# EdwardjkFeng/gradslam

Hardware: AMD Instinct MI355X
Metric: RGB-D frames/sec (640x480, 10 ICP iters) (higher is better)
Workload: dtype f32; 1 GPU; c2: ICP odometry localisation step, 640x480 TUM-shape synthetic RGB-D, batch 1 per GPU, dsratio 4 (~19k x ~19k points), 10 LM iterations, map 288269 points; parallelism=one sequence per GPU, final RCCL all_gather of poses, timing=one timed region of 1356 steps

## Files before the change

gradslam_amd/csrc/gs_drivers.hpp:

```cpp
#pragma once

#include "gs_common.hpp"
#include "gs_project.hpp"

namespace gs {

int vertex_normal_maps_cam(const float *depth, const float *intrinsics, const float *poses, int B, int H, int W, float *vertex,
                           float *normal, float *gvertex, float *gnormal, float *cam_out, hipStream_t st);
int vertex_normal_maps_fusion(const float *depth, const float *intrinsics, const float *poses, int B, int H, int W, float *gvertex,
                              float *gnormal, float *alpha, float sigma, float eps, unsigned long long *pix_key, unsigned int *pix_n,
                              int32_t *zero, int n_zero, hipStream_t st);

constexpr int kBucketPixMax = 24 * 1024;
size_t project_target1_ws_bytes(int H, int W, int ds, int Nmax);
int project_target1(const float *points, const int32_t *counts, int Nmax, const float *poses, const float *intrinsics, int H, int W, int ds,
                    const float *map_normals, int cap, int64_t *rows, int32_t *nrows, float *tgt, float *tnrm, int32_t *nt,
                    float *scan_points, int32_t *scan_orig, int32_t *pix_start, int32_t *tgt_index, int32_t *tgt_pix, void *ws,
                    size_t ws_bytes, hipStream_t st, const DsJob *frame);
int project_front1(const float *depth, const float *points, const int32_t *counts, int Nmax, const float *poses, const float *intrinsics,
                   int H, int W, int ds, const float *map_normals, int cap, float *vertex, float *normal, float *gvertex, float *gnormal,
                   float *cam_out, int32_t *row_pix, float *tgt, float *tnrm, int32_t *nt, int32_t *tgt_index, float *scan_points,
                   int32_t *scan_orig, int32_t *pix_start, const DsJob &frame, void *ws, size_t ws_bytes, hipStream_t st);

size_t fusion_corr_state_bytes(int B, int H, int W, int Nmax);
void fusion_corr_init_ptrs(void *state, int B, int H, int W, int Nmax, unsigned long long **pix_key, unsigned int **pix_n);
int fusion_correspond(void *state, const float *map_points, const float *map_normals, const float *map_ccounts, const int32_t *counts,
                      int B, int Nmax, const float *poses, const float *intrinsics, int H, int W, const float *gvertex,
                      const float *gnormal, float dist_th, float dot_th, int32_t *ctr, hipStream_t st);
int fusion_merge_corr(void *state, const int32_t *ctr, const float *gvertex, const float *gnormal, const float *rgb, const float *alpha,
                      int B, int H, int W, int Nmax, const int32_t *counts, float *points, float *normals, float *colors, float *ccounts,
                      hipStream_t st);
int fusion_append_corr(void *state, int B, int H, int W, int Nmax, int b, const float *depth, const float *const *h_src,
                       const int *h_row_floats, float *const *h_dst, const int32_t *d_count, int cap, int *d_total, void *cws,
                       hipStream_t st);
int fusion_finish(void *state, int B, int H, int W, int Nmax, int32_t *ctr, int32_t *counts, const int *totals, int cap, int32_t *appended,
                  int32_t *stats, hipStream_t st);
size_t append_scratch_bytes(int64_t HW);
size_t fusion_tape_bytes(int B, int H, int W);
int fusion_tape_record(const void *state, void *tape, int B, int H, int W, int Nmax, const int32_t *counts, const float *points,
                       const float *normals, const float *colors, const float *ccounts, hipStream_t st);
int fusion_tape_appended(void *tape, int B, int H, int W, const int32_t *appended, hipStream_t st);
int fusion_update_reverse(const void *tape, int B, int H, int W, int Nmax, const float *depth, const float *gvertex, const float *gnormal,
                          const float *rgb, const float *alpha, float *points, float *normals, float *colors, float *ccounts,
                          int32_t *counts, float *Gp, float *Gn, float *Gc, float *Gcc, float *g_gvertex, float *g_gnormal, float *g_rgb,
                          float *g_alpha, void *cws, hipStream_t st);
int append_valid_pixels(int n_arrays, const float *depth_b, int64_t HW, const float *const *h_src, const int *h_row_floats,
                        float *const *h_dst, int32_t *d_count, int cap, int32_t *d_appended, int32_t *d_overflow, void *cws,
                        hipStream_t st);

}
```

gradslam_amd/csrc/gs_icp_loop.hpp:

```cpp
#pragma once

#include "gs_icp_step.hpp"
#include "gs_project.hpp"

namespace gs {

struct LoopConst {
    const float *user_src, *tgt, *nrm, *boxes, *sboxes;
    const int32_t *d_ns, *d_nt;
    float *trace, *out_T;
    gs_icp_hints hints;
    GradParams gp;
    float thresh;
    int ns, nt;
    int cert_off;
    int tile_points;
    int grid_variant;
    CamK cam;
    int cam_ok;
    int32_t *cells;
    int cells_stride;
};

__device__ __forceinline__ f3 cam_point(const CamK &k, const f3 p) {
// ... 465 lines not shown
        unsigned long long scan_diag = 0;
#endif
        {
            float bd = INFINITY;
            int bi = 0x7fffffff;
            const int2 w0 = sh.wrow[0][lane], w1 = sh.wrow[1][lane], w2 = sh.wrow[2][lane];
            static_assert(WROWS == 3, "the flattened scan names its three rows");
            const int total = w0.y + w1.y + w2.y;
            auto element = [&](const int p) { return lanewin::element(p, w0.y, w1.y, w0.x, w1.x, w2.x); };
            auto take = [&](const float4 q) {
                const float d = dist2(s, q.x, q.y, q.z);
                const int jj = __float_as_int(q.w);
                const bool better = (d < bd) | ((d == bd) & (jj < bi));
                bd = better ? d : bd;
                bi = better ? jj : bi;
            };
#ifdef GS_DIAG_STAMPS
            unsigned int n_iter = 0;
#endif
            const float4 *pool = reinterpret_cast<const float4 *>(sh.u.stage);
            if (!__any((w0.x | w1.x | w2.x) < 0)) {
                for (int p = wave; p < total; p += 2 * NW) {
                    const int ea = element(p), eb = element(min(p + NW, total - 1));
                    const float4 qa = pool[ea], qb = pool[eb];
                    take(qa);
                    take(qb);
#ifdef GS_DIAG_STAMPS
                    ++n_iter;
#endif
                }
            } else {
                for (int p = wave; p < total; p += NW) {
                    const int e = element(p);
                    float4 q;
                    if (e >= 0) {
                        q = pool[e];
                    } else {
                        const int slot = LaneWin::mem_slot(e);
                        const f3 g3 = ld3(C->hints.scan_points, slot);
                        q = make_float4(g3.x, g3.y, g3.z, __int_as_float(C->hints.scan_orig[slot]));
                    }
                    take(q);
#ifdef GS_DIAG_STAMPS
                    ++n_iter;
#endif
                }
            }
            if (ok && bd < INFINITY) atomicMin(&sh.key[lane], pack_key(bd, bi));
#ifdef GS_DIAG_STAMPS
            scan_diag = ((unsigned long long)n_iter << 8) | ((unsigned long long)(unsigned)wave_max_i(total) << 32);
#endif
        }
        __syncthreads();
        GS_STAMP(1);
        float bd;
        int bi;
        key_unpack(sh.key[lane], bd, bi);
        const float bound2 = (ok && C->cam_ok) ? cam_bound2(sh.cam, s, sh.centre[lane], rel >> 3) : 0.0f;
        const bool proven = !C->cert_off & ((rel & 4) != 0) & (bd * 1.0001f < bound2);
        need = ok & !proven;
        unsigned long long need_mask = __ballot(need);
#ifdef GS_DIAG_STAMPS
        GS_COUNT(12, (unsigned long long)__popcll(need_mask) | scan_diag);
#endif
        if constexpr (NW == 8) {
            if (__popcll(need_mask) > 6 && C->cam_ok && !C->cert_off) {
                need = knn_second_window<NW>(sh, s, need, bd, nt, C->hints.pix_start, C->hints.scan_points, C->hints.scan_orig, win2_word);
                need_mask = __ballot(need);
            }
        }
        bool tile_search = __popcll(need_mask) > 6;
        if (!tile_search && need_mask) {
            tile_search = !knn_point_search<NW>(sh, s, need_mask, C->hints.scan_points, C->hints.scan_orig, C->boxes, C->sboxes, nt);
        }
        if (tile_search) {
            tile_box(sh, s, need);
            __syncthreads();
            knn_prune_search<true, NW>(sh, s, ok, need, C->hints.scan_points, C->hints.scan_orig, C->boxes, C->sboxes, nt);
        }
        if constexpr (NW == 8) win2_word |= (unsigned)__popcll(need_mask) | (tile_search ? 0x400u : 0u);
#ifdef GS_DIAG_STAMPS
        if (wave == 0) GS_COUNT(15, (unsigned long long)win2_word);
#endif

        GS_STAMP(2);
        key = ok ? sh.key[lane] : KEY_NONE;
        GS_STAMP(3);
        GS_COUNT(5, ((unsigned long long)__builtin_amdgcn_s_getreg((31 << 11) | 4) << 16) |
                        ((unsigned long long)__builtin_amdgcn_s_getreg((31 << 11) | 20) << 48));
    } else {
        int sj = -1;
        if (!first) {
            sj = -2;
            if (wave == 0) {
                unsigned long long k0 = KEY_NONE;
                if (ok) {
                    const float4 q = *reinterpret_cast<const float4 *>(sh.seed[b_cur == S_in->b_cur ? 0 : 1][lane]);
                    k0 = pack_key(dist2(s, q.x, q.y, q.z), __float_as_int(q.w));
                }
                sh.key[lane] = k0;
            }
        }
        const bool window_seed = first && C->hints.scan_points && C->hints.src_pix && C->hints.pix_start && C->hints.grid_w > 0;
        if (window_seed) sj = -2;
        const float *scan = C->hints.scan_points ? C->hints.scan_points : C->tgt;
        const int32_t *scan_orig = C->hints.scan_points ? C->hints.scan_orig : nullptr;
        if (window_seed) knn_window_seed<NW>(sh, s, ok, i, C->hints, nt);
        key = knn_tile<NW>(sh, s, ok, sj, C->tgt, scan, scan_orig, C->boxes, C->sboxes, nt);
    }
    if (wave == 0) {
        if (ok) best[i] = key;
        if (grid && ok && C->cam_ok) C->cells[par * C->cells_stride + i] = cam_cell(sh.cam, s);
        float acc[NACC];
#pragma unroll
        for (int k = 0; k < NACC; ++k) acc[k] = 0.0f;
        const Row r = make_row_from(s, ok, key, C->tgt, C->nrm, C->thresh);
        if (r.valid) accumulate_row(r, acc);
#pragma unroll
        for (int k = 0; k < NACC; ++k) sh.u.a.rows[k][lane] = acc[k];
    }
    __syncthreads();
    static_assert(NACC * 16 <= NW * 64, "the J epilogue's first stage is one pass");
    if (threadIdx.x < NACC * 16) {
        const int k = threadIdx.x >> 4, p4 = (threadIdx.x & 15) * 4;
        sh.u.a.part[k][threadIdx.x & 15] = ((sh.u.a.rows[k][p4] + sh.u.a.rows[k][p4 + 1]) + sh.u.a.rows[k][p4 + 2]) + sh.u.a.rows[k][p4 + 3];
    }
    __syncthreads();
    if (threadIdx.x < NACC) {
        float v = 0.0f;
#pragma unroll
        for (int q = 0; q < 16; ++q) v += sh.u.a.part[threadIdx.x][q];
        partials[blockIdx.x * NACC + threadIdx.x] = v;
    }
    if constexpr (GRID && NW == 8) {
        if (threadIdx.x == 0 && (win2_word & 0x300u)) window_count(win2_word);
    }
}

__global__ void icp_init_state_k(IcpState *S, const float *__restrict__ init_T , float damp) {
    if (threadIdx.x == 0 && blockIdx.x == 0) {
        for (int i = 0; i < 16; ++i) {
            const float v = init_T ? init_T[i] : ((i % 5 == 0) ? 1.0f : 0.0f);
            S->T[i] = v; S->dT[i] = v;
        }
        for (int i = 0; i < 44; ++i) S->cur[i] = 0.0f;
        S->damp = damp;
        S->p_cur = 1;
        S->b_cur = 1; S->b_first = 0;
        S->it = 0;
    }
}

__global__ __launch_bounds__(SUPER * CHUNK) void icp_prepare_k(IcpState *S, const float *__restrict__ init_T, float damp,
                                                              const float *__restrict__ tgt, const int32_t *__restrict__ d_nt,
                                                              float *__restrict__ boxes, float *__restrict__ sboxes,
                                                              LoopConst lc, LoopConst *__restrict__ lc_out, float *__restrict__ part0,
                                                              float *__restrict__ part1, int rows_written, int rows_read) {
    static_assert(SUPER * CHUNK == 1024, "one block per super-box");
    for (int q = rows_written * NACC + blockIdx.x * blockDim.x + threadIdx.x; q < rows_read * NACC; q += gridDim.x * blockDim.x) {
        part0[q] = 0.0f; part1[q] = 0.0f;
    }
    __shared__ float wb[16][6];
    if (blockIdx.x == 0 && threadIdx.x < sizeof(LoopConst) / 4) {
        int v = reinterpret_cast<const int *>(&lc)[threadIdx.x];
        if (threadIdx.x == offsetof(LoopConst, ns) / 4) v = *lc.d_ns;
        if (threadIdx.x == offsetof(LoopConst, nt) / 4) v = *lc.d_nt;
        if (threadIdx.x == offsetof(LoopConst, tile_points) / 4) {
            atomicAdd(&g_loop_counts[0], 1u);
            if (lc.grid_variant) atomicAdd(&g_loop_counts[1], 1u);
            if (lc.tile_points != 64) atomicAdd(&g_loop_counts[2], 1u);
        }
        reinterpret_cast<int *>(lc_out)[threadIdx.x] = v;
    }
    if (lc.cells) {
        const int n = *lc.d_ns;
        int32_t *pix = lc.cells + 2 * (size_t)lc.cells_stride;
        for (int i = blockIdx.x * blockDim.x + threadIdx.x; i < lc.cells_stride; i += gridDim.x * blockDim.x)
            pix[i] = (i < n && lc.hints.src_pix) ? lc.hints.src_pix[i] : 0;
    }
    if (blockIdx.x == 0) {
        __syncthreads();
        if (threadIdx.x == 0 && lc.hints.cam_pose && lc.hints.cam_K && lc.hints.ds > 0) {
            const float *T = lc.hints.cam_pose, *K = lc.hints.cam_K;
            const Cam c = make_cam(T, K);
            for (int q = 0; q < 9; ++q) lc_out->cam.R[q] = c.R[q];
            for (int q = 0; q < 3; ++q) lc_out->cam.T[q] = c.tinv[q];
            lc_out->cam.fx = K[0]; lc_out->cam.fy = K[5]; lc_out->cam.cx = K[2]; lc_out->cam.cy = K[6];
            lc_out->cam.ds = lc.hints.ds; lc_out->cam.Wd = lc.hints.grid_w; lc_out->cam.Hd = lc.hints.grid_h;
            const bool pinhole = K[1] == 0.0f && K[3] == 0.0f && K[4] == 0.0f && K[7] == 0.0f && K[8] == 0.0f && K[9] == 0.0f &&
                                 K[10] == 1.0f && K[11] == 0.0f && K[0] != 0.0f && K[5] != 0.0f;
            lc_out->cam_ok = pinhole ? 1 : 0;
        }
    }
    if (threadIdx.x == 0 && blockIdx.x == 0) {
        for (int i = 0; i < 16; ++i) {
            const float v = init_T ? init_T[i] : ((i % 5 == 0) ? 1.0f : 0.0f);
            S->T[i] = v; S->dT[i] = v;
        }
        for (int i = 0; i < 44; ++i) S->cur[i] = 0.0f;
        for (int i = 0; i < 6; ++i) S->xi[i] = 0.0f;
        S->damp = damp;
        S->p_cur = 1;
        S->b_cur = 1; S->b_first = 0;
        S->it = 0;
    }
    const int nt = *d_nt;
    const int j = blockIdx.x * (SUPER * CHUNK) + threadIdx.x;
    if (blockIdx.x * (SUPER * CHUNK) >= nt) return;
    float lo[3] = {INFINITY, INFINITY, INFINITY}, hi[3] = {-INFINITY, -INFINITY, -INFINITY};
    if (j < nt) {
        const f3 p = ld3(tgt, j);
        lo[0] = hi[0] = p.x; lo[1] = hi[1] = p.y; lo[2] = hi[2] = p.z;
    }
#pragma unroll
    for (int a = 0; a < 3; ++a) {
#pragma unroll
        for (int off = CHUNK / 2; off > 0; off >>= 1) {
            lo[a] = fminf(lo[a], __shfl_xor(lo[a], off, kWave));
            hi[a] = fmaxf(hi[a], __shfl_xor(hi[a], off, kWave));
        }
    }
    if ((threadIdx.x % CHUNK) == 0 && j < nt) {
        float *b = boxes + 6 * (int64_t)(j / CHUNK);
        b[0] = lo[0]; b[1] = lo[1]; b[2] = lo[2]; b[3] = hi[0]; b[4] = hi[1]; b[5] = hi[2];
    }
#pragma unroll
    for (int a = 0; a < 3; ++a) {
#pragma unroll
        for (int off = 32; off >= CHUNK; off >>= 1) {
            lo[a] = fminf(lo[a], __shfl_xor(lo[a], off, kWave));
            hi[a] = fmaxf(hi[a], __shfl_xor(hi[a], off, kWave));
        }
    }
    const int lane = threadIdx.x & 63, wave = threadIdx.x >> 6;
    if (lane == 0) { wb[wave][0] = lo[0]; wb[wave][1] = lo[1]; wb[wave][2] = lo[2]; wb[wave][3] = hi[0]; wb[wave][4] = hi[1]; wb[wave][5] = hi[2]; }
    __syncthreads();
    if (threadIdx.x < 6) {
        float v = wb[0][threadIdx.x];
        for (int w = 1; w < 16; ++w) v = threadIdx.x < 3 ? fminf(v, wb[w][threadIdx.x]) : fmaxf(v, wb[w][threadIdx.x]);
        sboxes[6 * (int64_t)blockIdx.x + threadIdx.x] = v;
    }
}

__global__ void copy_best_last_k(const IcpState *__restrict__ S, LoopBufs B, const int32_t *__restrict__ d_ns,
                                 unsigned long long *__restrict__ out) {
    const unsigned long long *src = B.N(S->b_first);
    const int ns = *d_ns;
    for (int i = blockIdx.x * blockDim.x + threadIdx.x; i < ns; i += gridDim.x * blockDim.x) out[i] = src[i];
}

}
```

gradslam_amd/csrc/gs_maps.hpp:

```cpp
#pragma once

#include "gs_common.hpp"

namespace gs {

constexpr int TW = 64, TH = 4;

struct Kinv4 {
    float a, c, e, f;
};

__device__ __forceinline__ Kinv4 load_kinv(const float *__restrict__ K) {
    const float eps = 1e-6f;
    const float fx = K[0] + eps, fy = K[5] + eps;
    return Kinv4{1.0f / fx, (-1.0f * K[2]) / fx, 1.0f / fy, (-1.0f * K[6]) / fy};
}

__device__ __forceinline__ f3 vertex_of(const Kinv4 k, int h, int w, float d) {
    const float m = d > 0.0f ? 1.0f : 0.0f;
    const float x = k.a * (float)w + k.c;
    const float y = k.e * (float)h + k.f;
    return f3{(x * d) * m, (y * d) * m, (1.0f * d) * m};
}

struct VnExtra {
    float *alpha;
    float alpha_den, alpha_eps;
    unsigned long long *pix_key;
    unsigned int *pix_n;
    int32_t *zero;
    int n_zero;
    float *cam_out;
};

__device__ __forceinline__ void vertex_normal_body(const float *__restrict__ depth, const float *__restrict__ Ks,
                                                   const float *__restrict__ poses, int L, int H, int W,
                                                   float *__restrict__ vertex, float *__restrict__ normal,
                                                   float *__restrict__ gvertex, float *__restrict__ gnormal, const VnExtra &ex,
                                                   int bx, int by, int bz) {
    __shared__ float sd[TH + 1][TW + 1];
    if (ex.zero && bx == 0 && by == 0 && bz == 0)
        for (int i = threadIdx.x; i < ex.n_zero; i += TW * TH) ex.zero[i] = 0;
    if (ex.cam_out && poses && bx == 0 && by == 0 && threadIdx.x < 32) {
        const int blz = bz;
        ex.cam_out[32 * blz + threadIdx.x] = threadIdx.x < 16 ? poses[16 * (int64_t)blz + threadIdx.x] : Ks[16 * (blz / L) + threadIdx.x - 16];
    }
    const int bl = bz;
    const int b = bl / L;
    const int w0 = bx * TW, h0 = by * TH;
    const int tx = threadIdx.x & (TW - 1), ty = threadIdx.x / TW;
    const float *dimg = depth + (int64_t)bl * H * W;

    for (int i = threadIdx.x; i < (TH + 1) * (TW + 1); i += TW * TH) {
        const int r = i / (TW + 1), c = i - r * (TW + 1);
        const int hh = min(h0 + r, H - 1), ww = min(w0 + c, W - 1);
        sd[r][c] = dimg[(int64_t)hh * W + ww];
    }
    __syncthreads();

    const int h = h0 + ty, w = w0 + tx;
    if (h >= H || w >= W) return;
    const Kinv4 k = load_kinv(Ks + 16 * b);
    const float d = sd[ty][tx];
    const f3 v = vertex_of(k, h, w, d);

    f3 dh, dv;
    if (w < W - 1) {
        const f3 vr = vertex_of(k, h, w + 1, sd[ty][tx + 1]);
        dh = f3{vr.x - v.x, vr.y - v.y, vr.z - v.z};
    } else {
        const float dl = (tx > 0) ? sd[ty][tx - 1] : dimg[(int64_t)h * W + (w - 1)];
        const f3 vl = vertex_of(k, h, w - 1, dl);
        dh = f3{v.x - vl.x, v.y - vl.y, v.z - vl.z};
    }
    if (h < H - 1) {
        const f3 vd = vertex_of(k, h + 1, w, sd[ty + 1][tx]);
        dv = f3{vd.x - v.x, vd.y - v.y, vd.z - v.z};
    } else {
        const float du = (ty > 0) ? sd[ty - 1][tx] : dimg[(int64_t)(h - 1) * W + w];
        const f3 vu = vertex_of(k, h - 1, w, du);
        dv = f3{v.x - vu.x, v.y - vu.y, v.z - vu.z};
    }
    f3 n;
    n.x = __fmaf_rn(dh.y, dv.z, -(dh.z * dv.y));
    n.y = __fmaf_rn(dh.z, dv.x, -(dh.x * dv.z));
    n.z = __fmaf_rn(dh.x, dv.y, -(dh.y * dv.x));
    float nn = sqrtf(__fmaf_rn(n.z, n.z, __fmaf_rn(n.y, n.y, n.x * n.x)));
    nn = (nn == 0.0f) ? 1.0f : nn;
    const float m = d > 0.0f ? 1.0f : 0.0f;
    n = f3{(n.x / nn) * m, (n.y / nn) * m, (n.z / nn) * m};

    const int64_t pix = (int64_t)bl * H * W + (int64_t)h * W + w;
    if (ex.alpha) {
        const float ss = (v.x * v.x + v.y * v.y) + v.z * v.z;
        ex.alpha[pix] = fminf(fmaxf(expf((-ss) / ex.alpha_den), ex.alpha_eps), 1.01f);
    }
    if (ex.pix_key) ex.pix_key[pix] = ~0ull;
    if (ex.pix_n) ex.pix_n[pix] = ~0u;
    if (vertex) st3(vertex, pix, v);
    if (normal) st3(normal, pix, n);
    if (gvertex || gnormal) {
        if (poses) {
            const float *T = poses + 16 * (int64_t)bl;
            if (gvertex) {
                f3 g = xform(T, v);
                st3(gvertex, pix, f3{g.x * m, g.y * m, g.z * m});
            }
            if (gnormal) {
                st3(gnormal, pix,
                    f3{dot3_fma(T[0], T[1], T[2], n.x, n.y, n.z), dot3_fma(T[4], T[5], T[6], n.x, n.y, n.z),
                       dot3_fma(T[8], T[9], T[10], n.x, n.y, n.z)});
            }
        } else {
            if (gvertex) st3(gvertex, pix, v);
            if (gnormal) st3(gnormal, pix, n);
        }
    }
}

}
```

gradslam_amd/csrc/gs_project.hpp:

```cpp
#pragma once

#include "gs_common.hpp"

namespace gs {

struct Cam {
    float R[9];
    float tinv[3];
    float K[16];
};

__device__ __forceinline__ Cam make_cam(const float *__restrict__ T, const float *__restrict__ K) {
    Cam c;
#pragma unroll
    for (int i = 0; i < 3; ++i)
#pragma unroll
        for (int j = 0; j < 3; ++j) c.R[3 * i + j] = T[4 * i + j];
    const float t0 = T[3], t1 = T[7], t2 = T[11];
#pragma unroll
    for (int j = 0; j < 3; ++j) c.tinv[j] = ((-T[j]) * t0 + (-T[4 + j]) * t1) + (-T[8 + j]) * t2;
#pragma unroll
    for (int i = 0; i < 16; ++i) c.K[i] = K[i];
    return c;
}
__device__ __forceinline__ void block_cam(Cam &cam, const float *__restrict__ poses, const float *__restrict__ Ks, int b) {
    if (threadIdx.x < 32) {
        const float w = threadIdx.x < 16 ? poses[16 * b + threadIdx.x] : Ks[16 * b + threadIdx.x - 16];
        __shared__ float raw[32];
        raw[threadIdx.x] = w;
        __builtin_amdgcn_wave_barrier();
        if (threadIdx.x == 0) cam = make_cam(raw, raw + 16);
    }
}
__device__ __forceinline__ bool project_point_z(const Cam &c, f3 p, int H, int W, float umax, float vmax, int &h, int &w, float &z) {
    const float x = dot3_fma(p.x, p.y, p.z, c.R[0], c.R[3], c.R[6]) + c.tinv[0];
    const float y = dot3_fma(p.x, p.y, p.z, c.R[1], c.R[4], c.R[7]) + c.tinv[1];
    z = dot3_fma(p.x, p.y, p.z, c.R[2], c.R[5], c.R[8]) + c.tinv[2];
    const bool front = z > 0.0f;
    const float *K = c.K;
    const float qx = ((K[0] * x + K[1] * y) + K[2] * z) + K[3] * 1.0f;
    const float qy = ((K[4] * x + K[5] * y) + K[6] * z) + K[7] * 1.0f;
    const float qz = ((K[8] * x + K[9] * y) + K[10] * z) + K[11] * 1.0f;
    const float zs = (qz != 0.0f) ? qz : 1.0f;
    const float u = qx / zs, v = qy / zs;
    const bool in = (u > -1e-3f) && (u < umax) && (v > -1e-3f) && (v < vmax) && front;
    const float ru = rintf(u), rv = rintf(v);
    w = (int)fminf(fmaxf(ru, 0.0f), (float)(W - 1));
    h = (int)fminf(fmaxf(rv, 0.0f), (float)(H - 1));
    return in;
}
__device__ __forceinline__ bool project_point(const Cam &c, f3 p, int H, int W, float umax, float vmax, int &h, int &w) {
    float z;
    return project_point_z(c, p, H, W, umax, vmax, h, w, z);
}


struct DsPred {
    const float *depth;
    int W, Wd, ds;
    __device__ bool operator()(int64_t i) const {
        const int r = (int)(i / Wd), c = (int)(i - (int64_t)r * Wd);
        return depth[(int64_t)(r * ds) * W + c * ds] > 0.0f;
    }
};
struct DsWriter {
    const float *gv, *gn, *rgb;
    float *op, *on, *oc;
    int32_t *opix;
    int W, Wd, ds;
    __device__ void operator()(int64_t i, int64_t pos) const {
        const int r = (int)(i / Wd), c = (int)(i - (int64_t)r * Wd);
        const int64_t pix = (int64_t)(r * ds) * W + c * ds;
        if (opix) opix[pos] = (int32_t)i;
        if (op) st3(op, pos, ld3(gv, pix));
        if (on) st3(on, pos, ld3(gn, pix));
        if (oc) st3(oc, pos, ld3(rgb, pix));
    }
};

struct DsJob {
    const float *depth, *gvertex;
    float *out_points;
    int32_t *out_pix;
    int32_t *count;
};

}
```

gradslam_amd/csrc/icp.hip:

```cpp
#include <stddef.h>
#include <stdlib.h>
#include <algorithm>
#include <vector>

#include "gs_detfold.hpp"
#include "gs_icp.hpp"
#include "gs_icp_reduce.hpp"
#include "gs_rowsum.hpp"

namespace gs {

__global__ __launch_bounds__(KNN_T) void knn1_brute_k(const float *__restrict__ src, const int32_t *__restrict__ d_ns,
                                                      const float *__restrict__ tgt, const int32_t *__restrict__ d_nt,
                                                      int nsplit, unsigned long long *__restrict__ best) {
    const int ns = *d_ns, nt = *d_nt;
    const int i = blockIdx.x * KNN_T + threadIdx.x;
    if (blockIdx.x * KNN_T >= ns) return;
    const int chunk = (nt + nsplit - 1) / nsplit;
    const int j0 = blockIdx.y * chunk, j1 = min(nt, j0 + chunk);
    const bool ok = i < ns;
    const f3 s = ok ? ld3(src, i) : f3{0.0f, 0.0f, 0.0f};
    float bd = INFINITY;
    int bi = 0;
    for (int j = j0; j < j1; ++j) {
// ... 136 lines not shown
        }
        if (g_tgt) {
            atomicAdd(g_tgt + 3 * (int64_t)j, bb * n.x);
            atomicAdd(g_tgt + 3 * (int64_t)j + 1, bb * n.y);
            atomicAdd(g_tgt + 3 * (int64_t)j + 2, bb * n.z);
        }
        if (g_nrm) {
            atomicAdd(g_nrm + 3 * (int64_t)j, nb.x);
            atomicAdd(g_nrm + 3 * (int64_t)j + 1, nb.y);
            atomicAdd(g_nrm + 3 * (int64_t)j + 2, nb.z);
        }
    }
}

__global__ void transform_k(const float *__restrict__ pts, const int32_t *__restrict__ d_n, const float *__restrict__ T,
                            float *__restrict__ out) {
    const int n = *d_n;
    for (int i = blockIdx.x * blockDim.x + threadIdx.x; i < n; i += gridDim.x * blockDim.x) st3(out, i, xform(T, ld3(pts, i)));
}

}

#include "gs_icp_loop.hpp"
#include "gs_icp_bwd.hpp"

namespace gs {

static inline int knn_nsplit_brute(int max_ns, int max_nt) {
    const int tiles = cdiv(max_ns, KNN_T);
    int ns = cdiv(2048, tiles);
    const int cap = cdiv(max_nt, 64);
    if (ns > cap) ns = cap;
    if (ns < 1) ns = 1;
    if (ns > 4096) ns = 4096;
    return ns;
}
static inline int lin_blocks(int max_ns) {
    int nb = cdiv(max_ns, LIN_T);
    if (nb > LIN_MAXB) nb = LIN_MAXB;
    if (nb < 1) nb = 1;
    return nb;
}
static inline size_t boxes_bytes(int max_nt) { return (size_t)cdiv(max_nt > 0 ? max_nt : 1, CHUNK) * 6 * 4; }

struct Prof {
    bool on = false;
    std::vector<hipEvent_t> ev[2][2];
    size_t used[2] = {0, 0};
    double total_ms[2] = {0.0, 0.0};
    long count[2] = {0, 0};
};
static Prof g_prof;
static inline void prof_mark(int tag, int which, hipStream_t st) {
    if (!g_prof.on) return;
    auto &v = g_prof.ev[tag][which];
    const size_t i = g_prof.used[tag];
    if (i >= v.size()) {
        hipEvent_t e;
        if (hipEventCreate(&e) != hipSuccess) return;
        v.push_back(e);
    }
    (void)hipEventRecord(v[i], st);
    if (which == 1) g_prof.used[tag] = i + 1;
}

bool profiling_enabled() { return g_prof.on; }

static int g_grid_mode = getenv("GS_GRID_MODE") ? atoi(getenv("GS_GRID_MODE")) : 1;
static int g_tile_points = 0;
static int g_loop_waves = 0;

constexpr int TILE_MIN = 32;
static inline int loop_tile_points() {
    static const int env = getenv("GS_TILE_POINTS") ? atoi(getenv("GS_TILE_POINTS")) : 0;
    const int forced = g_tile_points ? g_tile_points : env;
    return (forced >= TILE_MIN && forced <= 64) ? forced : 64;
}
constexpr int LOOP_WAVES_DENSE = 64;
static inline int loop_waves(bool grid_search, int max_nt, int cells) {
    static const int env = getenv("GS_LOOP_WAVES") ? atoi(getenv("GS_LOOP_WAVES")) : 0;
    const int forced = g_loop_waves ? g_loop_waves : env;
    if (forced == 8 || forced == 16) return forced;
    return (grid_search && (int64_t)max_nt <= (int64_t)LOOP_WAVES_DENSE * cells) ? 8 : 16;
}
int icp_config_stamp() { return g_grid_mode | (g_tile_points << 4) | (g_loop_waves << 12); }
static inline int loop_blocks_max(int max_ns) { return cdiv(max_ns, TILE_MIN); }
static inline int partial_rows_alloc(int max_ns) { return std::max(loop_blocks_max(max_ns), 32 * RP_LOADS) + 1; }

struct IcpWs {
    IcpState *S[2];
    LoopBufs B;
    float *partials[2];
    float *boxes, *sboxes;
    LoopConst *lc;
    int32_t *cells;
};
template <class T>
static inline T *take_slots(Carve &c, int n, size_t bytes, int64_t *stride) {
    const size_t o = c.off;
    T *first = c.take<T>(bytes);
    *stride = (int64_t)((c.off - o) / sizeof(T));
    for (int k = 1; k < n; ++k) c.take(bytes);
    return first;
}
static inline size_t icp_ws_layout(int max_ns, int max_nt, void *ws, IcpWs *out) {
    Carve c{(char *)ws};
    IcpWs scratch, &w = out ? *out : scratch;
    const size_t part_b = (size_t)partial_rows_alloc(max_ns) * NACC * 4;
    w.S[0] = c.take<IcpState>(sizeof(IcpState)); w.S[1] = c.take<IcpState>(sizeof(IcpState));
    w.B.pts = take_slots<float>(c, 2, (size_t)max_ns * 12, &w.B.pts_stride);
    w.B.best = take_slots<unsigned long long>(c, 2, (size_t)max_ns * 8, &w.B.best_stride);
    w.partials[0] = c.take<float>(part_b); w.partials[1] = c.take<float>(part_b);
    w.boxes = c.take<float>(boxes_bytes(max_nt));
    w.sboxes = c.take<float>((size_t)cdiv(max_nt > 0 ? max_nt : 1, 1024) * 6 * 4);
    w.lc = c.take<LoopConst>(sizeof(LoopConst));
    w.cells = c.take<int32_t>((size_t)max_ns * 12);
    return c.off;
}

struct Tape {
    float *rec;
    LoopBufs B;
    int nslots;
};
static inline int tape_launches(bool grad, int numiters) { return grad ? 2 * numiters : numiters + 1; }
static inline size_t tape_layout(bool grad, int max_ns, int numiters, void *tape, Tape *out) {
    Carve c{(char *)tape};
    Tape scratch, &t = out ? *out : scratch;
    t.nslots = tape_launches(grad, numiters > 0 ? numiters : 1);
    t.rec = c.take<float>((size_t)(t.nslots + 1) * REC_WORDS * 4);
    t.B.pts = take_slots<float>(c, t.nslots, (size_t)max_ns * 12, &t.B.pts_stride);
    t.B.best = take_slots<unsigned long long>(c, t.nslots, (size_t)max_ns * 8, &t.B.best_stride);
    return c.off;
}

static inline GradParams make_grad_params(float lambda_max, float B, float B2, float nu) {
    return GradParams{(float)(1.0 / (double)lambda_max), (float)((double)lambda_max - 1.0 / (double)lambda_max), B, B2,
                      (float)(1.0 / (double)nu)};
}
static inline GradParams lm_grad_params() { return GradParams{0.5f, 1.5f, 1.0f, 1.0f, 0.005f}; }

__global__ __launch_bounds__(1024) void icp_step_k(IcpState *__restrict__ Sg, const float *__restrict__ partials, int nblocks,
                                                  int mode, GradParams gp, float *__restrict__ trace ,
                                                  float *__restrict__ out_T, int look_slot,
                                                  float *__restrict__ rec , int solve,
                                                  const float *__restrict__ compose_right, float *__restrict__ compose_out) {
    __shared__ float acc[NACC];
    __shared__ double lu_sm[42];
    __shared__ IcpState st;
    constexpr int kWords = sizeof(IcpState) / 4;
#ifdef GS_DIAG_STAMPS
    if (g_diag && threadIdx.x == 0) g_diag[0] = wall_clock64();
#endif
    if (threadIdx.x < kWords) reinterpret_cast<int *>(&st)[threadIdx.x] = reinterpret_cast<const int *>(Sg)[threadIdx.x];
    reduce_partials(partials, nblocks, acc);
    if (rec && threadIdx.x < kWords) reinterpret_cast<int *>(rec)[REC_STATE + threadIdx.x] = reinterpret_cast<const int *>(Sg)[threadIdx.x];
#ifdef GS_DIAG_STAMPS
    if (g_diag && threadIdx.x == 0) g_diag[1] = wall_clock64();
#endif
    if (threadIdx.x < 64) step_wave0(&st, acc, mode, gp, trace, out_T, look_slot, rec, lu_sm, solve != 0);
#ifdef GS_DIAG_STAMPS
    if (g_diag && threadIdx.x == 0) g_diag[2] = wall_clock64();
#endif
    __syncthreads();
    if (threadIdx.x < kWords) {
        const int v = reinterpret_cast<const int *>(&st)[threadIdx.x];
        reinterpret_cast<int *>(Sg)[threadIdx.x] = v;
        if (rec) reinterpret_cast<int *>(rec)[REC_WORDS + REC_STATE + threadIdx.x] = v;
    }
    if (compose_out && threadIdx.x == 0) compose44(st.T, compose_right, compose_out);
}

static int icp_run(bool grad, const float *src, const int32_t *d_ns, int max_ns, const float *tgt, const float *nrm,
                   const int32_t *d_nt, int max_nt, const float *init_T, int numiters, float damp, float thresh,
                   GradParams gp, const gs_icp_hints *hints_in, float *out_T, uint64_t *best_last, float *trace, void *ws,
                   size_t ws_bytes, hipStream_t st, const char *name, void *tape = nullptr, size_t tape_bytes = 0,
                   const float *compose_right = nullptr, float *compose_out = nullptr) {
    gs_icp_hints hints{nullptr, nullptr, nullptr, nullptr, nullptr, 0, 0, nullptr, nullptr, 0};
    if (hints_in) hints = *hints_in;
    GS_REQUIRE(!hints.scan_points || hints.scan_orig, "%s: hints.scan_points needs hints.scan_orig", name);
    GS_REQUIRE(src && d_ns && tgt && nrm && d_nt && out_T, "%s: NULL argument", name);
    GS_REQUIRE(max_ns > 0 && max_nt > 0 && numiters >= 0, "%s: bad sizes max_ns=%d max_nt=%d numiters=%d", name, max_ns, max_nt, numiters);
    IcpWs w;
    GS_REQUIRE_WS(name, ws, ws_bytes, icp_ws_layout(max_ns, max_nt, ws, &w));
    if (numiters == 0) {
        if (init_T) {
            GS_HIP(hipMemcpyAsync(out_T, init_T, 64, hipMemcpyDeviceToDevice, st), name);
        } else {
            hipLaunchKernelGGL(icp_init_state_k, dim3(1), dim3(64), 0, st, w.S[0], init_T, damp);
            GS_HIP(hipMemcpyAsync(out_T, w.S[0], 64, hipMemcpyDeviceToDevice, st), name);
        }
        return GS_OK;
    }
    Tape tp{nullptr, {}, 0};
    if (tape) {
        GS_REQUIRE_TAPE(name, tape, tape_bytes, tape_layout(grad, max_ns, numiters, tape, &tp), GS_ERR_WORKSPACE_TOO_SMALL);
        w.B = tp.B;
    }
    int n_assoc = 0, n_step = 0;
    const int tile_points = loop_tile_points();
    const dim3 kgrid(cdiv(max_ns, tile_points));
    const int lb = (int)kgrid.x;
    const int fb = min(cdiv(max_ns, 256), 256);

    static const int cert_off = getenv("GS_CERT_OFF") != nullptr;
    static const bool grid_off = getenv("GS_NO_GRID_SEARCH") != nullptr;
    const bool grid_search = !grid_off && g_grid_mode != 0 && hints.scan_points && hints.scan_orig && hints.src_pix && hints.pix_start &&
                             hints.cam_pose && hints.cam_K && hints.ds > 0 && hints.grid_w > 0 && hints.grid_h > 0;
    LoopConst lc{src, tgt, nrm, w.boxes, w.sboxes, d_ns, d_nt, trace, out_T, hints, gp, thresh, 0, 0, cert_off, tile_points,
                 grid_search ? 1 : 0, CamK{}, 0, w.cells, max_ns};
    hipLaunchKernelGGL(icp_prepare_k, dim3(cdiv(max_nt, SUPER * CHUNK)), dim3(SUPER * CHUNK), 0, st, w.S[0], init_T, damp,
                       hints.scan_points ? hints.scan_points : tgt, d_nt, w.boxes, w.sboxes, lc, w.lc, w.partials[0], w.partials[1], lb,
                       std::max(lb, 32 * RP_LOADS));
    GS_LAUNCH_CHECK(name);
    int cur = 0;
    int pending = -1;
    int pending_slot = -1;
    const bool fold = (int)kgrid.x <= 2 * 256;
    auto assoc = [&](int first) {
        if (!fold && pending >= 0) {
            hipLaunchKernelGGL(icp_step_k, dim3(1), dim3(1024), 0, st, w.S[cur], w.partials[cur], lb, pending, gp, trace, out_T,
                               pending_slot, tape ? tp.rec + (size_t)n_step * REC_WORDS : nullptr, 1, (const float *)nullptr,
                               (float *)nullptr);
            ++n_step;
            pending = -1;
        }
        const int nxt = pending >= 0 ? 1 - cur : cur;
        prof_mark(0, 0, st);
        float *rec_p = (tape && pending >= 0) ? tp.rec + (size_t)n_step * REC_WORDS : nullptr;
        const int nw = loop_waves(grid_search, max_nt, hints.grid_w * hints.grid_h);
        auto launch_nw = [&](auto kernel, int waves) {
            hipLaunchKernelGGL(kernel, kgrid, dim3(waves * 64), 0, st, (const LoopConst *)w.lc, (const IcpState *)w.S[cur], (const float *)w.partials[cur],
                               (const int32_t *)(w.cells + 2 * (size_t)max_ns), (const int32_t *)(w.cells + (size_t)(1 - (n_assoc & 1)) * max_ns),
                               max_ns, tile_points, first | ((n_assoc & 1) << 1), pending, pending_slot, lb, w.S[nxt], rec_p,
                               tape ? n_assoc : -1, w.B, w.partials[nxt], src);
        };
        auto launch = [&](auto k16, auto k8) {
            if (nw == 16) launch_nw(k16, 16); else launch_nw(k8, 8);
        };
        if (grid_search && lb <= 32 * RP_FEW) launch(knn1_loop_k<true, RP_FEW, 16>, knn1_loop_k<true, RP_FEW, 8>);
        else if (grid_search) launch(knn1_loop_k<true, RP_LOADS, 16>, knn1_loop_k<true, RP_LOADS, 8>);
        else launch(knn1_loop_k<false, RP_LOADS, 16>, knn1_loop_k<false, RP_LOADS, 8>);
        prof_mark(0, 1, st);
        if (pending >= 0) ++n_step;
        cur = nxt;
        pending = -1;
        ++n_assoc;
    };
    auto step = [&](int mode) {
        pending = mode;
        pending_slot = tape ? n_assoc - 1 : -1;
    };
    auto finish = [&]() {
        hipLaunchKernelGGL(icp_step_k, dim3(1), dim3(1024), 0, st, w.S[cur], w.partials[cur], lb, pending, gp, trace, out_T,
                           pending_slot, tape ? tp.rec + (size_t)n_step * REC_WORDS : nullptr, 0, compose_right, compose_out);
        ++n_step;
        pending = -1;
    };
    assoc(1);
    step(STEP_ADOPT);
    if (!grad) {
        for (int it = 0; it < numiters; ++it) {
            assoc(0);
            step(STEP_LM);
        }
    } else {
        for (int it = 0; it < numiters; ++it) {
            assoc(0);
            step(STEP_GRAD_B);
            if (it + 1 < numiters) {
                assoc(0);
                step(STEP_ADOPT);
            }
        }
    }
    finish();
    GS_LAUNCH_CHECK(name);
    if (best_last) {
        hipLaunchKernelGGL(copy_best_last_k, dim3(fb), dim3(256), 0, st, w.S[cur], w.B, d_ns, (unsigned long long *)best_last);
        GS_LAUNCH_CHECK(name);
    }
    return GS_OK;
}

static inline int bwd_launches(bool grad, int numiters) { return grad ? 2 * numiters : numiters; }
struct BwdDetWs {
    BwdWs bwd;
    DetWs det;
};
static inline size_t bwd_det_layout(bool det, bool grad, int max_ns, int max_nt, int numiters, void *ws, BwdDetWs *out) {
    Carve c{(char *)ws};
    BwdDetWs scratch, &w = out ? *out : scratch;
    bwd_ws_layout(max_ns, c.take(bwd_ws_layout(max_ns, nullptr, nullptr)), &w.bwd);
    w.det = DetWs{};
    if (det) {
        const int Q = bwd_launches(grad, numiters > 0 ? numiters : 1);
        det_ws_layout(Q, max_ns, max_nt, c.take(det_ws_layout(Q, max_ns, max_nt, nullptr, nullptr)), &w.det);
    }
    return c.off;
}

static int icp_backward_run(bool grad, const float *src, const int32_t *d_ns, int max_ns, const float *tgt, const float *nrm,
                            const int32_t *d_nt, int max_nt, const float *init_T, int numiters, float thresh, GradParams gp, const void *tape,
                            size_t tape_bytes, const float *grad_T, float *g_src, float *g_tgt, float *g_nrm, float *g_init_T,
                            void *ws, size_t ws_bytes, hipStream_t st, bool det = false) {
    const char *name = det ? "gs_icp_backward_det" : "gs_icp_backward";
    GS_REQUIRE(src && d_ns && tgt && nrm && d_nt && init_T && tape && grad_T && g_src && g_init_T, "%s: NULL argument", name);
    GS_REQUIRE(max_ns > 0 && max_nt > 0 && numiters >= 0, "%s: bad sizes", name);
    GS_REQUIRE(!det || bwd_launches(grad, numiters) <= 65535, "%s: too many iterations for the deterministic fold", name);
    BwdDetWs both;
    GS_REQUIRE_WS(name, ws, ws_bytes, bwd_det_layout(det, grad, max_ns, max_nt, numiters, ws, &both));
    Tape tp;
    GS_REQUIRE_TAPE(name, tape, tape_bytes, tape_layout(grad, max_ns, numiters, (void *)tape, &tp), GS_ERR_INVALID_ARG);
    const BwdWs &w = both.bwd;
    const DetWs &dw = both.det;
    const bool fold = det && (g_tgt || g_nrm);
    auto rows_of = [&](int q) { return fold ? dw.rows + (size_t)q * max_ns * DET_ROW : nullptr; };
    float *walk_nrm = det ? nullptr : g_nrm;
    const int nb = min(cdiv(max_ns, BWD_T), BWD_MAXB);
    int cur = 0;
    hipLaunchKernelGGL(bwd_begin_k, dim3(min(cdiv(3 * max(max_nt, max_ns), 256), 1024)), dim3(256), 0, st, w.S[0], grad_T, w.gP, 3 * max_ns,
                       w.partials[0], nb * 12, det ? nullptr : g_tgt, walk_nrm, d_nt, max_nt);
    for (int k = numiters - 1, q = 0; k >= 0; --k) {
        if (!grad) {
            const float *rec = tp.rec + (size_t)(1 + k) * REC_WORDS;
            float *gt = det ? rows_of(q++) : g_tgt;
            hipLaunchKernelGGL(det ? bwd_lin_k<true> : bwd_lin_k<false>, dim3(nb), dim3(BWD_T), 0, st, (const BwdState *)w.S[cur],
                               w.S[1 - cur], (int)FOLD_LM, rec, (const float *)w.partials[cur], nb, k, 1, tp.B, src, d_ns, tgt, nrm, thresh,
                               w.gP, gt, walk_nrm, w.partials[1 - cur]);
            cur = 1 - cur;
        } else {
            const float *rec = tp.rec + (size_t)(1 + 2 * k) * REC_WORDS;
            float *gt = det ? rows_of(q++) : g_tgt;
            hipLaunchKernelGGL(det ? bwd_look_k<true> : bwd_look_k<false>, dim3(nb), dim3(BWD_T), 0, st, (const BwdState *)w.S[cur],
                               w.S[1 - cur], rec, (const float *)w.partials[cur], nb, gp, k == 0 ? -1 : (k == 1 ? 0 : 2 * (k - 1)), tp.B, d_ns,
                               tgt, nrm, thresh, w.gP, gt, walk_nrm, w.partials[1 - cur]);
            cur = 1 - cur;
            gt = det ? rows_of(q++) : g_tgt;
            hipLaunchKernelGGL(det ? bwd_lin_k<true> : bwd_lin_k<false>, dim3(nb), dim3(BWD_T), 0, st, (const BwdState *)w.S[cur],
                               w.S[1 - cur], (int)FOLD_G2, rec, (const float *)w.partials[cur], nb, 0, 0, tp.B, src, d_ns, tgt, nrm, thresh,
                               w.gP, gt, walk_nrm, w.partials[1 - cur]);
            cur = 1 - cur;
        }
    }
    hipLaunchKernelGGL(bwd_finish_k, dim3(nb), dim3(BWD_T), 0, st, init_T, d_ns, (const float *)w.gP, g_src, (const BwdState *)w.S[cur],
                       (const float *)w.partials[cur], nb, g_init_T);
    GS_LAUNCH_CHECK(name);
    if (fold) return det_fold_run(dw, bwd_launches(grad, numiters), max_ns, d_ns, d_nt, max_nt, g_tgt, g_nrm, st, name);
    return GS_OK;
}

int icp_localize_run(int grad_lm, const float *src, const int32_t *d_ns, int max_ns, const float *tgt, const float *nrm,
                     const int32_t *d_nt, int max_nt, int numiters, float damp, float thresh, float lambda_max, float Bp,
                     float B2, float nu, const gs_icp_hints *hints, float *out_T, void *ws, size_t ws_bytes, hipStream_t st,
                     void *tape, size_t tape_bytes, const float *compose_right, float *compose_out) {
    const GradParams gp = grad_lm ? make_grad_params(lambda_max, Bp, B2, nu) : lm_grad_params();
    return icp_run(grad_lm != 0, src, d_ns, max_ns, tgt, nrm, d_nt, max_nt, nullptr, numiters, damp, thresh, gp, hints, out_T, nullptr,
                   nullptr, ws, ws_bytes, st, "gs_slam_localize/icp", tape, tape_bytes, compose_right, compose_out);
}

}

using namespace gs;

extern "C" {
// ... 272 lines not shown
```

gradslam_amd/csrc/maps.hip:

```cpp
#include <stdarg.h>

#include "gs_common.hpp"
#include "gs_compact.hpp"
#include "gs_drivers.hpp"
#include "gs_maps.hpp"
#include "gs_project.hpp"
#include "gs_rowsum.hpp"

namespace gs {

static thread_local char g_err[512] = "";
void set_error(const char *fmt, ...) {
    va_list ap;
    va_start(ap, fmt);
    vsnprintf(g_err, sizeof(g_err), fmt, ap);
    va_end(ap);
}

__global__ __launch_bounds__(TW *TH) void vertex_normal_k(const float *__restrict__ depth, const float *__restrict__ Ks,
                                                          const float *__restrict__ poses, int L, int H, int W,
                                                          float *__restrict__ vertex, float *__restrict__ normal,
                                                          float *__restrict__ gvertex, float *__restrict__ gnormal, VnExtra ex) {
    vertex_normal_body(depth, Ks, poses, L, H, W, vertex, normal, gvertex, gnormal, ex, (int)blockIdx.x, (int)blockIdx.y, (int)blockIdx.z);
}
// ... 371 lines not shown
    return GS_OK;
}

int gs_vertex_normal_maps_backward(const float *depth, const float *intrinsics, const float *poses, int B, int L, int H,
                                   int W, const float *g_vertex, const float *g_normal, const float *g_gvertex,
                                   const float *g_gnormal, float *g_depth, float *g_intrinsics, float *g_poses,
                                   void *ws, size_t ws_bytes, gs_stream_t stream) {
    return maps_backward(false, depth, intrinsics, poses, B, L, H, W, g_vertex, g_normal, g_gvertex, g_gnormal, g_depth, g_intrinsics,
                         g_poses, ws, ws_bytes, stream);
}

int gs_vertex_normal_maps_backward_det(const float *depth, const float *intrinsics, const float *poses, int B, int L, int H,
                                       int W, const float *g_vertex, const float *g_normal, const float *g_gvertex,
                                       const float *g_gnormal, float *g_depth, float *g_intrinsics, float *g_poses,
                                       void *ws, size_t ws_bytes, gs_stream_t stream) {
    return maps_backward(true, depth, intrinsics, poses, B, L, H, W, g_vertex, g_normal, g_gvertex, g_gnormal, g_depth, g_intrinsics,
                         g_poses, ws, ws_bytes, stream);
}

int gs_get_alpha(const float *points, int64_t n, float sigma, float eps, float *alpha, gs_stream_t stream) {
    GS_REQUIRE(points && alpha && n >= 0, "gs_get_alpha: bad arguments");
    if (n == 0) return GS_OK;
    const float den = 2.0f * (sigma * sigma);
    hipLaunchKernelGGL(alpha_k, dim3(min(cdiv(n, 256), 4096)), dim3(256), 0, (hipStream_t)stream, points, n, den, eps, alpha);
    GS_LAUNCH_CHECK("gs_get_alpha");
    return GS_OK;
}

int gs_get_alpha_backward(const float *points, int64_t n, float sigma, float eps, const float *g_alpha, float *g_points,
                          gs_stream_t stream) {
    GS_REQUIRE(points && g_alpha && g_points && n >= 0, "gs_get_alpha_backward: bad arguments");
    if (n == 0) return GS_OK;
    const float den = 2.0f * (sigma * sigma);
    hipLaunchKernelGGL(alpha_bwd_k, dim3(min(cdiv(n, 256), 4096)), dim3(256), 0, (hipStream_t)stream, points, n, den, eps,
                       g_alpha, g_points);
    GS_LAUNCH_CHECK("gs_get_alpha_backward");
    return GS_OK;
}

size_t gs_compact_ws_bytes(int64_t n_rows) { return compact_ws_bytes(n_rows); }

int gs_compact_rows(const float *src, const uint8_t *mask, int64_t n_rows, int row_floats, float *out,
                    int32_t *out_count, void *ws, size_t ws_bytes, gs_stream_t stream) {
    GS_REQUIRE(mask && out_count && n_rows >= 0 && row_floats >= 0, "gs_compact_rows: bad arguments");
    GS_REQUIRE(row_floats == 0 || (src && out), "gs_compact_rows: src/out must not be NULL when row_floats > 0");
    GS_REQUIRE_WS("gs_compact_rows", ws, ws_bytes, compact_ws_bytes(n_rows));
    MaskPred pred{mask};
    RowWriter wr{(const uint32_t *)src, (uint32_t *)out, row_floats};
    return compact_launch(n_rows, pred, wr, out_count, ws, (hipStream_t)stream, "gs_compact_rows");
}

int gs_compact_multi(int n_arrays, const float *const *h_src, const int *h_row_floats, float *const *h_out,
                     const uint8_t *mask, int64_t n_rows, int32_t *out_count, void *ws, size_t ws_bytes,
                     gs_stream_t stream) {
    GS_REQUIRE(n_arrays >= 1 && n_arrays <= 4 && h_src && h_row_floats && h_out && mask && out_count && n_rows >= 0,
               "gs_compact_multi: bad arguments (1..4 arrays)");
    GS_REQUIRE_WS("gs_compact_multi", ws, ws_bytes, compact_ws_bytes(n_rows));
    MultiWriter wr;
    wr.n_arrays = n_arrays;
    for (int a = 0; a < 4; ++a) {
        wr.src[a] = a < n_arrays ? (const uint32_t *)h_src[a] : nullptr;
        wr.out[a] = a < n_arrays ? (uint32_t *)h_out[a] : nullptr;
        wr.words[a] = a < n_arrays ? h_row_floats[a] : 0;
        GS_REQUIRE(a >= n_arrays || (h_src[a] && h_out[a] && h_row_floats[a] > 0), "gs_compact_multi: NULL array %d", a);
    }
    MaskPred pred{mask};
    return compact_launch(n_rows, pred, wr, out_count, ws, (hipStream_t)stream, "gs_compact_multi");
}

int gs_expand_multi(int n_arrays, const float *const *h_grad, const int *h_row_floats, float *const *h_out,
                    const uint8_t *mask, int64_t n_rows, void *ws, size_t ws_bytes, gs_stream_t stream) {
    GS_REQUIRE(n_arrays >= 1 && n_arrays <= 4 && h_grad && h_row_floats && h_out && mask && n_rows >= 0,
               "gs_expand_multi: bad arguments (1..4 arrays)");
    GS_REQUIRE_WS("gs_expand_multi", ws, ws_bytes, compact_ws_bytes(n_rows));
    ExpandWriter wr;
    wr.n_arrays = n_arrays;
    for (int a = 0; a < 4; ++a) {
        wr.g[a] = a < n_arrays ? (const uint32_t *)h_grad[a] : nullptr;
        wr.out[a] = a < n_arrays ? (uint32_t *)h_out[a] : nullptr;
        wr.words[a] = a < n_arrays ? h_row_floats[a] : 0;
        GS_REQUIRE(a >= n_arrays || (h_grad[a] && h_out[a] && h_row_floats[a] > 0), "gs_expand_multi: NULL array %d", a);
    }
    MaskPred pred{mask};
    return compact_launch(n_rows, pred, wr, (int *)nullptr, ws, (hipStream_t)stream, "gs_expand_multi");
}

int gs_frames_from_raw(const uint16_t *depth_raw, const uint8_t *rgb_raw, int B, int Hs, int Ws, int Hd, int Wd,
                       float depth_scale, int normalise_color, float *depth, float *rgb, gs_stream_t stream) {
    GS_REQUIRE(B > 0 && B <= 65535 && Hs > 0 && Ws > 0 && Hd > 0 && Wd > 0, "gs_frames_from_raw: bad shape");
    GS_REQUIRE((!depth_raw || depth) && (!rgb_raw || rgb) && (depth_raw || rgb_raw), "gs_frames_from_raw: NULL output for a given input");
    GS_REQUIRE(!depth_raw || depth_scale > 0.0f, "gs_frames_from_raw: depth_scale must be positive");
    hipLaunchKernelGGL(frames_from_raw_k, dim3(min(cdiv((int64_t)Hd * Wd, 256), 2048), B), dim3(256), 0, (hipStream_t)stream,
                       depth_raw, rgb_raw, Hs, Ws, Hd, Wd, (double)depth_scale, normalise_color, depth, rgb);
    GS_LAUNCH_CHECK("gs_frames_from_raw");
    return GS_OK;
}

size_t gs_append_rows_ws_bytes(int64_t n_rows) { return compact_layout(n_rows, true, nullptr, nullptr); }

int gs_append_rows(int n_arrays, const float *const *h_src, const int *h_row_floats, float *const *h_dst, const uint8_t *mask,
                   int64_t n_rows, int32_t *d_count, int cap, int32_t *d_appended, int32_t *d_overflow, void *ws,
                   size_t ws_bytes, gs_stream_t stream) {
    GS_REQUIRE(n_arrays >= 1 && n_arrays <= 4 && h_src && h_row_floats && h_dst && mask && d_count && n_rows >= 0 && cap >= 0,
               "gs_append_rows: bad arguments (1..4 arrays)");
    GS_REQUIRE_WS("gs_append_rows", ws, ws_bytes, gs_append_rows_ws_bytes(n_rows));
    AppendWriter wr;
    wr.n_arrays = n_arrays;
    wr.base = d_count;
    wr.cap = cap;
    for (int a = 0; a < 4; ++a) {
        wr.src[a] = a < n_arrays ? (const uint32_t *)h_src[a] : nullptr;
        wr.out[a] = a < n_arrays ? (uint32_t *)h_dst[a] : nullptr;
        wr.words[a] = a < n_arrays ? h_row_floats[a] : 0;
        GS_REQUIRE(a >= n_arrays || (h_src[a] && h_dst[a] && h_row_floats[a] > 0), "gs_append_rows: NULL array %d", a);
    }
    int *total = compact_ws(n_rows, true, ws).total;
    MaskPred pred{mask};
    const int rc = compact_launch(n_rows, pred, wr, total, ws, (hipStream_t)stream, "gs_append_rows");
    if (rc) return rc;
    hipLaunchKernelGGL(append_count_k, dim3(1), dim3(64), 0, (hipStream_t)stream, d_count, total, cap, d_appended, d_overflow);
    GS_LAUNCH_CHECK("gs_append_rows/count");
    return GS_OK;
}

size_t gs_downsample_frame_ws_bytes(int H, int W, int ds) {
    return compact_ws_bytes((int64_t)cdiv(H, ds) * cdiv(W, ds));
}

int gs_downsample_frame(const float *depth, const float *gvertex, const float *gnormal, const float *rgb, int B, int H,
                        int W, int ds, int cap, float *out_points, float *out_normals, float *out_colors,
                        int32_t *out_pix, int32_t *counts, void *ws, size_t ws_bytes, gs_stream_t stream) {
    GS_REQUIRE(depth && counts && B > 0 && H > 0 && W > 0 && ds > 0, "gs_downsample_frame: bad arguments");
    const int Hd = cdiv(H, ds), Wd = cdiv(W, ds);
    GS_REQUIRE(cap >= Hd * Wd, "gs_downsample_frame: cap (%d) < ceil(H/ds)*ceil(W/ds) (%d)", cap, Hd * Wd);
    GS_REQUIRE((!out_points || gvertex) && (!out_normals || gnormal) && (!out_colors || rgb),
               "gs_downsample_frame: an output was requested without its source map");
    GS_REQUIRE_WS("gs_downsample_frame", ws, ws_bytes, gs_downsample_frame_ws_bytes(H, W, ds));
    const int64_t HW = (int64_t)H * W;
    for (int b = 0; b < B; ++b) {
        DsPred pred{depth + b * HW, W, Wd, ds};
        DsWriter wr{gvertex ? gvertex + 3 * b * HW : nullptr, gnormal ? gnormal + 3 * b * HW : nullptr,
                    rgb ? rgb + 3 * b * HW : nullptr,
                    out_points ? out_points + 3 * (int64_t)b * cap : nullptr,
                    out_normals ? out_normals + 3 * (int64_t)b * cap : nullptr,
                    out_colors ? out_colors + 3 * (int64_t)b * cap : nullptr,
                    out_pix ? out_pix + (int64_t)b * cap : nullptr, W, Wd, ds};
        int rc = compact_launch((int64_t)Hd * Wd, pred, wr, counts + b, ws, (hipStream_t)stream, "gs_downsample_frame");
        if (rc != GS_OK) return rc;
    }
    return GS_OK;
}

}
```

gradslam_amd/csrc/project.hip:

```cpp
#include "gs_common.hpp"
#include "gs_compact.hpp"
#include "gs_drivers.hpp"
#include "gs_maps.hpp"
#include "gs_project.hpp"

namespace gs {

constexpr int kCamB = 32;
__device__ __forceinline__ Cam *cam_cache() {
    __shared__ Cam cams[kCamB];
    return cams;
}

__global__ void build_cams_k(const float *__restrict__ poses, const float *__restrict__ Ks, int B, Cam *__restrict__ cams) {
    const int b = blockIdx.x * blockDim.x + threadIdx.x;
    if (b >= B) return;
    const float *T = poses + 16 * b;
    Cam c;
#pragma unroll
    for (int i = 0; i < 3; ++i)
#pragma unroll
        for (int j = 0; j < 3; ++j) c.R[3 * i + j] = T[4 * i + j];
    const float t0 = T[3], t1 = T[7], t2 = T[11];
#pragma unroll
    for (int j = 0; j < 3; ++j) {
        c.tinv[j] = ((-T[j]) * t0 + (-T[4 + j]) * t1) + (-T[8 + j]) * t2;
    }
#pragma unroll
    for (int i = 0; i < 16; ++i) c.K[i] = Ks[16 * b + i];
    cams[b] = c;
}

struct ActivePred {
    const float *points;
    const int32_t *counts;
    const Cam *cams;
    int Nmax, H, W, ds;
    float umax, vmax;
    __device__ bool operator()(int64_t i) const {
        const int b = (int)(i / Nmax), n = (int)(i - (int64_t)b * Nmax);
        if (n >= counts[b]) return false;
        int h, w;
        if (!project_point(cams[b], ld3(points, i), H, W, umax, vmax, h, w)) return false;
        return ds <= 0 || ((h % ds == 0) && (w % ds == 0));
    }
};
struct ActiveWriter {
    const float *points;
    const Cam *cams;
    int64_t *rows;
    int Nmax, H, W;
    float umax, vmax;
    __device__ void operator()(int64_t i, int64_t pos) const {
        const int b = (int)(i / Nmax), n = (int)(i - (int64_t)b * Nmax);
        int h, w;
        project_point(cams[b], ld3(points, i), H, W, umax, vmax, h, w);
        st_table_row(rows, pos, b, n, h, w);
    }
};

struct ActivePredL {
    const float *points;
    const int32_t *counts;
    const float *poses, *Ks;
    int B, Nmax, H, W, ds;
    float umax, vmax;
    __device__ void block_init(int , int , int ) const {
        for (int b = threadIdx.x; b < B; b += blockDim.x) cam_cache()[b] = make_cam(poses + 16 * b, Ks + 16 * b);
    }
    struct Item { f3 p; };
    __device__ Item fetch(int64_t i) const { return Item{ld3(points, i)}; }
    __device__ bool test(const Item &it, int64_t i) const {
        const int b = (int)(i / Nmax), n = (int)(i - (int64_t)b * Nmax);
        if (n >= counts[b]) return false;
        int h, w;
        if (!project_point(cam_cache()[b], it.p, H, W, umax, vmax, h, w)) return false;
        return ds <= 0 || ((h % ds == 0) && (w % ds == 0));
    }
    __device__ bool operator()(int64_t i) const { return test(fetch(i), i); }
};
struct ActiveWriterL {
    const float *points;
    int64_t *rows;
    int Nmax, H, W;
    float umax, vmax;
    __device__ void put(const ActivePredL::Item &it, int64_t i, int64_t pos) const {
        const int b = (int)(i / Nmax), n = (int)(i - (int64_t)b * Nmax);
        int h, w;
        project_point(cam_cache()[b], it.p, H, W, umax, vmax, h, w);
        longlong4 r;
        r.x = b; r.y = n; r.z = h; r.w = w;
        st_table_row(rows, pos, r);
    }
    __device__ void operator()(int64_t i, int64_t pos) const { put(ActivePredL::Item{ld3(points, i)}, i, pos); }
};

struct ActivePredH {
    const float *points;
    const int32_t *counts;
    const float *poses, *Ks;
    int Nmax, H, W, ds;
    float umax, vmax;
    int *cnt, *fill;
    int npix;
    __device__ void block_init(int pass, int bid, int nb) const {
        if (threadIdx.x == 0) cam_cache()[0] = make_cam(poses, Ks);
        if (pass == 0)
            for (int i = bid * blockDim.x + threadIdx.x; i < npix; i += nb * blockDim.x) { cnt[i] = 0; fill[i] = 0; }
    }
    struct Item { f3 p; };
    __device__ Item fetch(int64_t i) const { return Item{ld3(points, i)}; }
    __device__ bool test(const Item &it, int64_t i) const {
        if (i >= counts[0]) return false;
        int h, w;
        if (!project_point(cam_cache()[0], it.p, H, W, umax, vmax, h, w)) return false;
        return (h % ds == 0) && (w % ds == 0);
    }
    __device__ bool operator()(int64_t i) const { return test(fetch(i), i); }
};
struct ActiveWriterH {
    const float *points;
    int64_t *rows;
    int H, W, ds, Wd;
    float umax, vmax;
    int *cnt;
    __device__ void put(const ActivePredH::Item &it, int64_t i, int64_t pos) const {
        int h, w;
        project_point(cam_cache()[0], it.p, H, W, umax, vmax, h, w);
        st_table_row(rows, pos, 0, i, h, w);
        atomicAdd(cnt + (h / ds) * Wd + (w / ds), 1);
    }
    __device__ void operator()(int64_t i, int64_t pos) const { put(ActivePredH::Item{ld3(points, i)}, i, pos); }
};

struct ActiveWriterT {
    const float *points, *normals;
    int H, W, ds, Wd;
    float umax, vmax;
    int *cnt;
    int cap;
    float *tgt, *tnrm;
    int32_t *tgt_index;
    int32_t *row_pix;
    __device__ void put(const ActivePredH::Item &it, int64_t i, int64_t pos) const {
        int h, w;
        project_point(cam_cache()[0], it.p, H, W, umax, vmax, h, w);
        const int pix = (h / ds) * Wd + (w / ds);
        atomicAdd(cnt + pix, 1);
        row_pix[pos] = pix;
        if (pos < cap) {
            st3(tgt, pos, it.p);
            st3(tnrm, pos, ld3(normals, i));
            if (tgt_index) tgt_index[pos] = (int32_t)i;
        }
    }
    __device__ void operator()(int64_t i, int64_t pos) const { put(ActivePredH::Item{ld3(points, i)}, i, pos); }
};

__global__ void table_starts_k(const int64_t *__restrict__ rows, const int32_t *__restrict__ d_n, int B, int32_t *__restrict__ starts) {
    const int b = blockIdx.x * blockDim.x + threadIdx.x;
    if (b > B) return;
    const int n = *d_n;
    int lo = 0, hi = n;
    while (lo < hi) {
        const int mid = (lo + hi) >> 1;
        if (rows[4 * (int64_t)mid] < b) lo = mid + 1; else hi = mid;
    }
    starts[b] = lo;
}

__global__ void gather_table_k(const int64_t *__restrict__ rows, const int32_t *__restrict__ d_n,
                               const int32_t *__restrict__ starts, const float *__restrict__ attr, int B, int Nmax, int C,
                               int cap, float *__restrict__ out, int32_t *__restrict__ counts) {
    const int n = *d_n;
    if (blockIdx.x == 0 && threadIdx.x < B && counts) counts[threadIdx.x] = starts[threadIdx.x + 1] - starts[threadIdx.x];
    for (int64_t i = (int64_t)blockIdx.x * blockDim.x + threadIdx.x; i < n; i += (int64_t)gridDim.x * blockDim.x) {
        const int b = (int)rows[4 * i], p = (int)rows[4 * i + 1];
        const int k = (int)(i - starts[b]);
        if (k >= cap) continue;
        const float *s = attr + ((int64_t)b * Nmax + p) * C;
        float *d = out + ((int64_t)b * cap + k) * C;
        for (int c = 0; c < C; ++c) d[c] = s[c];
    }
}

__global__ void table_ds_mask_k(const int64_t *__restrict__ rows, int64_t n, int ds, uint8_t *__restrict__ mask) {
    for (int64_t i = (int64_t)blockIdx.x * blockDim.x + threadIdx.x; i < n; i += (int64_t)gridDim.x * blockDim.x)
        mask[i] = ((rows[4 * i + 2] % ds) == 0 && (rows[4 * i + 3] % ds) == 0) ? 1 : 0;
}

__global__ void pix_count_k(const int64_t *__restrict__ rows, const int32_t *__restrict__ d_n,
                            const int32_t *__restrict__ starts, int Wd, int npix, int ds, int *__restrict__ cnt) {
    const int n = *d_n;
    for (int64_t i = (int64_t)blockIdx.x * blockDim.x + threadIdx.x; i < n; i += (int64_t)gridDim.x * blockDim.x) {
        const longlong4 r = ld_table_row(rows, i);
        const int b = (int)r.x;
        const int pix = (int)(r.z / ds) * Wd + (int)(r.w / ds);
        atomicAdd(cnt + (int64_t)b * npix + pix, 1);
    }
}
constexpr int PIX_TILE = 24 * 1024;
__global__ __launch_bounds__(1024) void pix_scan_k(const int *__restrict__ cnt, int npix, int *__restrict__ start) {
    __shared__ int sm[1024 / 64 + 1];
    __shared__ int bins[PIX_TILE];
    __shared__ int carry;
    const int b = blockIdx.x;
    cnt += (int64_t)b * npix; start += (int64_t)b * (npix + 1);
    if (threadIdx.x == 0) carry = 0;
    __syncthreads();
    for (int t0 = 0; t0 < npix; t0 += PIX_TILE) {
        const int nb = min(PIX_TILE, npix - t0);
        for (int i = threadIdx.x; i < nb; i += 1024) bins[i] = cnt[t0 + i];
        __syncthreads();
        const int per = (nb + 1023) / 1024;
        const int i0 = min(nb, (int)threadIdx.x * per), i1 = min(nb, i0 + per);
        int sum = 0;
        for (int i = i0; i < i1; ++i) sum += bins[i];
        int total;
        int run = carry + block_excl_scan<1024>(sum, sm, &total);
        for (int i = i0; i < i1; ++i) { const int c = bins[i]; bins[i] = run; run += c; }
        __syncthreads();
        for (int i = threadIdx.x; i < nb; i += 1024) start[t0 + i] = bins[i];
        if (threadIdx.x == 0) carry += total;
        __syncthreads();
    }
    if (threadIdx.x == 0) start[npix] = carry;
}
__global__ void pix_scatter_k(const int64_t *__restrict__ rows, const int32_t *__restrict__ d_n,
                              const int32_t *__restrict__ starts, int Wd, int npix, int ds,
                              const int *__restrict__ start, int *__restrict__ fill, const float *__restrict__ map_points,
                              int Nmax, int cap, float *__restrict__ scan_pts, int32_t *__restrict__ scan_orig,
                              int32_t *__restrict__ tgt_pix ) {
    const int n = *d_n;
    for (int64_t i = (int64_t)blockIdx.x * blockDim.x + threadIdx.x; i < n; i += (int64_t)gridDim.x * blockDim.x) {
        const longlong4 r = ld_table_row(rows, i);
        const int b = (int)r.x;
        const int pix = (int)(r.z / ds) * Wd + (int)(r.w / ds);
        const int k = (int)(i - starts[b]);
        if (tgt_pix && k < cap) tgt_pix[(int64_t)b * cap + k] = pix;
        const int slot = start[(int64_t)b * (npix + 1) + pix] + atomicAdd(fill + (int64_t)b * npix + pix, 1);
        if (slot >= cap) continue;
        st3(scan_pts, (int64_t)b * cap + slot, ld3(map_points, (int64_t)b * Nmax + r.y));
        scan_orig[(int64_t)b * cap + slot] = (int32_t)k;
    }
}
__global__ void tgt_init_k(int *__restrict__ cnt, int *__restrict__ fill, int64_t n, const int64_t *__restrict__ rows,
                           const int32_t *__restrict__ d_n, int B, int32_t *__restrict__ starts) {
    for (int64_t i = (int64_t)blockIdx.x * blockDim.x + threadIdx.x; i < n; i += (int64_t)gridDim.x * blockDim.x) {
        cnt[i] = 0; fill[i] = 0;
    }
    if (blockIdx.x == 0) {
        for (int b = threadIdx.x; b <= B; b += blockDim.x) {
            int lo = 0, hi = *d_n;
            while (lo < hi) {
                const int mid = (lo + hi) >> 1;
                if (rows[4 * (int64_t)mid] < b) lo = mid + 1; else hi = mid;
            }
            starts[b] = lo;
        }
    }
}
__global__ void tgt_gather_count_k(const int64_t *__restrict__ rows, const int32_t *__restrict__ d_n,
                                   const int32_t *__restrict__ starts, const float *__restrict__ map_points,
                                   const float *__restrict__ map_normals, int B, int Nmax, int cap,
                                   float *__restrict__ tgt, float *__restrict__ tnrm, int32_t *__restrict__ counts, int Wd,
                                   int npix, int ds, int *__restrict__ cnt, int32_t *__restrict__ tgt_index) {
    const int n = *d_n;
    if (blockIdx.x == 0 && threadIdx.x < B) counts[threadIdx.x] = starts[threadIdx.x + 1] - starts[threadIdx.x];
    for (int64_t i = (int64_t)blockIdx.x * blockDim.x + threadIdx.x; i < n; i += (int64_t)gridDim.x * blockDim.x) {
        const longlong4 r = ld_table_row(rows, i);
        const int b = (int)r.x;
        const int k = (int)(i - starts[b]);
        const int pix = (int)(r.z / ds) * Wd + (int)(r.w / ds);
        atomicAdd(cnt + (int64_t)b * npix + pix, 1);
        if (k >= cap) continue;
        const int64_t src = (int64_t)b * Nmax + r.y, dst = (int64_t)b * cap + k;
        st3(tgt, dst, ld3(map_points, src));
        st3(tnrm, dst, ld3(map_normals, src));
        if (tgt_index) tgt_index[dst] = (int32_t)r.y;
    }
}

__global__ void tgt_scatter_gather1_k(const int64_t *__restrict__ rows, const int32_t *__restrict__ d_n,
                                      const float *__restrict__ map_points, const float *__restrict__ map_normals, int cap,
                                      float *__restrict__ tgt, float *__restrict__ tnrm, int32_t *__restrict__ counts,
                                      int32_t *__restrict__ tgt_index, int Wd, int ds, const int *__restrict__ start,
                                      int *__restrict__ fill, float *__restrict__ scan_pts, int32_t *__restrict__ scan_orig,
                                      int32_t *__restrict__ tgt_pix ) {
    const int n = *d_n;
    if (blockIdx.x == 0 && threadIdx.x == 0) counts[0] = n;
    for (int64_t i = (int64_t)blockIdx.x * blockDim.x + threadIdx.x; i < n; i += (int64_t)gridDim.x * blockDim.x) {
        const longlong4 r = ld_table_row(rows, i);
        const f3 p = ld3(map_points, r.y);
        if (i < cap) {
            st3(tgt, i, p);
            st3(tnrm, i, ld3(map_normals, r.y));
            if (tgt_index) tgt_index[i] = (int32_t)r.y;
        }
        const int pix = (int)(r.z / ds) * Wd + (int)(r.w / ds);
        if (tgt_pix && i < cap) tgt_pix[i] = pix;
        const int slot = start[pix] + atomicAdd(fill + pix, 1);
        if (slot >= cap) continue;
        st3(scan_pts, slot, p);
        scan_orig[slot] = (int32_t)i;
    }
}

struct ActiveWs {
    Cam *cams;
    void *cws;
};
static size_t active_layout(int B, int Nmax, void *ws, ActiveWs *out) {
    Carve c{(char *)ws};
    ActiveWs scratch, &w = out ? *out : scratch;
    w.cams = c.take<Cam>(sizeof(Cam) * (size_t)(B > 0 ? B : 1));
    w.cws = c.take(compact_ws_bytes((int64_t)B * Nmax));
    return c.off;
}

struct FrontWs {
    int *cnt, *fill;
    void *map_cws;
    unsigned char *flags;
    void *frame_cws;
};
static size_t front_layout(int H, int W, int ds, int Nmax, void *ws, FrontWs *out) {
    const size_t npix = (size_t)cdiv(H, ds) * cdiv(W, ds);
    Carve c{(char *)ws};
    FrontWs scratch, &w = out ? *out : scratch;
    w.cnt = c.take<int>(npix * 4); w.fill = c.take<int>(npix * 4);
    w.map_cws = c.take(compact_ws_bytes(Nmax));
    w.flags = c.take<unsigned char>(compact_flags_bytes(Nmax));
    w.frame_cws = c.take(compact_ws_bytes((int64_t)npix));
    return c.off;
}

struct BucketWs {
    int32_t *starts;
    int *cnt, *fill;
};
static size_t bucket_layout(int B, int H, int W, int ds, void *ws, BucketWs *out) {
    const size_t npix = (size_t)cdiv(H, ds) * cdiv(W, ds);
    Carve c{(char *)ws};
    BucketWs scratch, &w = out ? *out : scratch;
    w.starts = c.take<int32_t>(sizeof(int32_t) * (size_t)(B + 1));
    w.cnt = c.take<int>((size_t)B * npix * 4); w.fill = c.take<int>((size_t)B * npix * 4);
    return c.off;
}

}

using namespace gs;

extern "C" {

size_t gs_project_active_ws_bytes(int B, int Nmax) { return active_layout(B, Nmax, nullptr, nullptr); }

int gs_project_active(const float *points, const int32_t *counts, int B, int Nmax, const float *poses,
                      const float *intrinsics, int H, int W, int ds, int64_t *out_rows, int32_t *out_count, void *ws,
                      size_t ws_bytes, gs_stream_t stream) {
    GS_REQUIRE(points && counts && poses && intrinsics && out_rows && out_count, "gs_project_active: NULL argument");
    GS_REQUIRE(B > 0 && Nmax > 0 && H > 0 && W > 0, "gs_project_active: bad shape B=%d Nmax=%d H=%d W=%d", B, Nmax, H, W);
    ActiveWs w;
    GS_REQUIRE_WS("gs_project_active", ws, ws_bytes, active_layout(B, Nmax, ws, &w));
    hipStream_t st = (hipStream_t)stream;
    const float umax = (float)((double)W - 0.999), vmax = (float)((double)H - 0.999);
    if (B <= kCamB) {
        ActivePredL pred{points, counts, poses, intrinsics, B, Nmax, H, W, ds, umax, vmax};
        ActiveWriterL wr{points, out_rows, Nmax, H, W, umax, vmax};
        return compact_launch((int64_t)B * Nmax, pred, wr, out_count, w.cws, st, "gs_project_active");
    }
    hipLaunchKernelGGL(build_cams_k, dim3(cdiv(B, 64)), dim3(64), 0, st, poses, intrinsics, B, w.cams);
    GS_LAUNCH_CHECK("gs_project_active/cams");
    ActivePred pred{points, counts, w.cams, Nmax, H, W, ds, umax, vmax};
    ActiveWriter wr{points, w.cams, out_rows, Nmax, H, W, umax, vmax};
    return compact_launch((int64_t)B * Nmax, pred, wr, out_count, w.cws, st, "gs_project_active");
}

}

namespace gs {
size_t project_target1_ws_bytes(int H, int W, int ds, int Nmax) { return front_layout(H, W, ds, Nmax, nullptr, nullptr); }
int project_target1(const float *points, const int32_t *counts, int Nmax, const float *poses, const float *intrinsics, int H,
                    int W, int ds, const float *map_normals, int cap, int64_t *rows, int32_t *nrows, float *tgt, float *tnrm,
                    int32_t *nt, float *scan_points, int32_t *scan_orig, int32_t *pix_start, int32_t *tgt_index, int32_t *tgt_pix,
                    void *ws, size_t ws_bytes, hipStream_t st, const DsJob *frame) {
    const char *name = "gs_slam_localize/target";
    FrontWs w;
    GS_REQUIRE_WS(name, ws, ws_bytes, front_layout(H, W, ds, Nmax, ws, &w));
    const int Wd = cdiv(W, ds), npix = cdiv(H, ds) * Wd;
    int *cnt = w.cnt, *fill = w.fill;
    void *cws = w.map_cws, *dws = w.frame_cws;
    unsigned char *flags = w.flags;
    const float umax = (float)((double)W - 0.999), vmax = (float)((double)H - 0.999);
    ActivePredH pred{points, counts, poses, intrinsics, Nmax, H, W, ds, umax, vmax, cnt, fill, npix};
    ActiveWriterH wr{points, rows, H, W, ds, Wd, umax, vmax, cnt};
    int rc;
    if (frame) {
        const int Hd = cdiv(H, ds);
        DsPred dp{frame->depth, W, Wd, ds};
        DsWriter dw{frame->gvertex, nullptr, nullptr, frame->out_points, nullptr, nullptr, frame->out_pix, W, Wd, ds};
        if (compact_blocks((int64_t)Hd * Wd) <= kSelfScanBlocks) {
            rc = compact_launch2((int64_t)Nmax, pred, wr, nrows, cws, flags, (int64_t)Hd * Wd, dp, dw, frame->count, dws, st, name);
        } else {
            rc = compact_launch((int64_t)Hd * Wd, dp, dw, frame->count, dws, st, name);
            if (rc == GS_OK) rc = compact_launch((int64_t)Nmax, pred, wr, nrows, cws, st, name, flags);
        }
    } else {
        rc = compact_launch((int64_t)Nmax, pred, wr, nrows, cws, st, name, flags);
    }
    if (rc) return rc;
    hipLaunchKernelGGL(pix_scan_k, dim3(1), dim3(1024), 0, st, cnt, npix, pix_start);
    hipLaunchKernelGGL(tgt_scatter_gather1_k, dim3(min(cdiv(Nmax, 256), 1024)), dim3(256), 0, st, rows, nrows, points, map_normals, cap,
                       tgt, tnrm, nt, tgt_index, Wd, ds, pix_start, fill, scan_points, scan_orig, tgt_pix);
    GS_LAUNCH_CHECK(name);
    return GS_OK;
}

template <class PA, class PB>
__global__ __launch_bounds__(kCT) void setup_count_k(int64_t nA, PA pa, int *__restrict__ countsA, unsigned char *__restrict__ flagsA, int nbA,
                                                     int64_t nB, PB pb, int *__restrict__ countsB, int nbB, const float *__restrict__ depth,
                                                     const float *__restrict__ Ks, const float *__restrict__ poses, int H, int W, int gx,
                                                     float *__restrict__ vertex, float *__restrict__ normal, float *__restrict__ gvertex,
                                                     float *__restrict__ gnormal, VnExtra ex) {
    static_assert(kCT == TW * TH, "one block size for all three jobs");
    const int bid = (int)blockIdx.x;
    if (bid < nbA) {
        compact_count_body(nA, pa, countsA, flagsA, bid, nbA);
    } else if (bid < nbA + nbB) {
        compact_count_body(nB, pb, countsB, (unsigned char *)nullptr, bid - nbA, nbB);
    } else {
        const int t = bid - nbA - nbB;
        vertex_normal_body(depth, Ks, poses, 1, H, W, vertex, normal, gvertex, gnormal, ex, t % gx, t / gx, 0);
    }
}

constexpr int kBucketBlocks = 128;
__global__ __launch_bounds__(1024) void bucket_scatter_k(const float *__restrict__ tgt, const int32_t *__restrict__ d_nt, int cap,
                                                         const int32_t *__restrict__ row_pix, const int *__restrict__ cnt,
                                                         int *__restrict__ fill, int npix, int32_t *__restrict__ pix_start,
                                                         float *__restrict__ scan_pts, int32_t *__restrict__ scan_orig) {
    __shared__ int starts[kBucketPixMax];
    __shared__ int sm[1024 / 64 + 1];
    const int nt = *d_nt;
    for (int i = threadIdx.x; i < npix; i += 1024) starts[i] = cnt[i];
    const int stride = gridDim.x * 1024;
    int r = blockIdx.x * 1024 + threadIdx.x, pix = 0;
    f3 p{0.0f, 0.0f, 0.0f};
    if (r < nt) { pix = row_pix[r]; p = ld3(tgt, r); }
    __syncthreads();
    const int per = (npix + 1023) / 1024;
    const int i0 = min(npix, (int)threadIdx.x * per), i1 = min(npix, i0 + per);
    int sum = 0;
    for (int i = i0; i < i1; ++i) sum += starts[i];
    int total;
    int run = block_excl_scan<1024>(sum, sm, &total);
    for (int i = i0; i < i1; ++i) { const int c = starts[i]; starts[i] = run; run += c; }
    __syncthreads();
    if (blockIdx.x == 0) {
        for (int i = threadIdx.x; i < npix; i += 1024) pix_start[i] = starts[i];
        if (threadIdx.x == 0) pix_start[npix] = total;
    }
    for (; r < nt; r += stride) {
        const int slot = starts[pix] + atomicAdd(fill + pix, 1);
        const int rn = r + stride;
        int pn = 0;
        f3 pp{0.0f, 0.0f, 0.0f};
        if (rn < nt) { pn = row_pix[rn]; pp = ld3(tgt, rn); }
        if (slot < cap) {
            st3(scan_pts, slot, p);
            scan_orig[slot] = r;
        }
        pix = pn; p = pp;
    }
}

int project_front1(const float *depth, const float *points, const int32_t *counts, int Nmax, const float *poses, const float *intrinsics,
                   int H, int W, int ds, const float *map_normals, int cap, float *vertex, float *normal, float *gvertex, float *gnormal,
                   float *cam_out, int32_t *row_pix, float *tgt, float *tnrm, int32_t *nt, int32_t *tgt_index, float *scan_points,
                   int32_t *scan_orig, int32_t *pix_start, const DsJob &frame, void *ws, size_t ws_bytes, hipStream_t st) {
    const char *name = "gs_slam_localize/front";
    FrontWs w;
    GS_REQUIRE_WS(name, ws, ws_bytes, front_layout(H, W, ds, Nmax, ws, &w));
    const int Wd = cdiv(W, ds), Hd = cdiv(H, ds), npix = Hd * Wd;
    if (npix > kBucketPixMax) {
        set_error("%s: ds-grid too large for the fused form", name);
        return GS_ERR_INVALID_ARG;
    }
    int *cnt = w.cnt, *fill = w.fill;
    unsigned char *flags = w.flags;
    const float umax = (float)((double)W - 0.999), vmax = (float)((double)H - 0.999);
    ActivePredH pa{points, counts, poses, intrinsics, Nmax, H, W, ds, umax, vmax, cnt, fill, npix};
    ActiveWriterT wa{points, map_normals, H, W, ds, Wd, umax, vmax, cnt, cap, tgt, tnrm, tgt_index, row_pix};
    DsPred pb{frame.depth, W, Wd, ds};
    DsWriter wb{frame.gvertex, nullptr, nullptr, frame.out_points, nullptr, nullptr, frame.out_pix, W, Wd, ds};
    const int64_t nA = Nmax, nB = (int64_t)npix;
    const CompactWs cA = compact_ws(nA, false, w.map_cws);
    int *countsA = cA.counts, *countsB = compact_ws(nB, false, w.frame_cws).counts;
    const int nbA = compact_blocks(nA), nbB = compact_blocks(nB), gx = cdiv(W, TW), nbV = depth ? gx * cdiv(H, TH) : 0;
    if (nbB > kSelfScanBlocks) {
        set_error("%s: ds-grid too large for the fused form", name);
        return GS_ERR_INVALID_ARG;
    }
    const VnExtra ex{nullptr, 1.0f, 0.0f, nullptr, nullptr, nullptr, 0, cam_out};
    hipLaunchKernelGGL((setup_count_k<ActivePredH, DsPred>), dim3(nbA + nbB + nbV), dim3(kCT), 0, st, nA, pa, countsA, flags, nbA, nB, pb,
                       countsB, nbB, depth, intrinsics, poses, H, W, gx, vertex, normal, gvertex, gnormal, ex);
    GS_LAUNCH_CHECK(name);
    if (nbA <= kSelfScanBlocks) {
        hipLaunchKernelGGL((compact_write2_k<ActivePredH, ActiveWriterT, true, DsPred, DsWriter>), dim3(nbA + nbB), dim3(kCT), 0, st, nA, pa, wa,
                           (const int *)countsA, nt, (const unsigned char *)flags, nbA, nB, pb, wb, (const int *)countsB, frame.count, nbB);
    } else {
        int *offsetsA = cA.offsets;
        hipLaunchKernelGGL(compact_scan_k, dim3(1), dim3(1024), 0, st, countsA, nbA, offsetsA, nt);
        GS_LAUNCH_CHECK(name);
        hipLaunchKernelGGL((compact_write2_k<ActivePredH, ActiveWriterT, false, DsPred, DsWriter>), dim3(nbA + nbB), dim3(kCT), 0, st, nA, pa, wa,
                           (const int *)offsetsA, (int *)nullptr, (const unsigned char *)flags, nbA, nB, pb, wb, (const int *)countsB,
                           frame.count, nbB);
    }
    GS_LAUNCH_CHECK(name);
    hipLaunchKernelGGL(bucket_scatter_k, dim3(std::min(cdiv(cap, 1024), kBucketBlocks)), dim3(1024), 0, st, (const float *)tgt,
                       (const int32_t *)nt, cap, (const int32_t *)row_pix, (const int *)cnt, fill, npix, pix_start, scan_points, scan_orig);
    GS_LAUNCH_CHECK(name);
    return GS_OK;
}
}

extern "C" {

size_t gs_gather_table_rows_ws_bytes(int B) { return one_piece_bytes(sizeof(int32_t) * (size_t)(B + 1)); }

int gs_gather_table_rows(const int64_t *rows, const int32_t *d_n_rows, int64_t max_rows, const float *attr, int B,
                         int Nmax, int C, int cap, float *out, int32_t *counts, void *ws, size_t ws_bytes,
                         gs_stream_t stream) {
    GS_REQUIRE(rows && d_n_rows && attr && out, "gs_gather_table_rows: NULL argument");
    GS_REQUIRE(B > 0 && B <= 256 && Nmax > 0 && C > 0 && cap >= 0 && max_rows >= 0, "gs_gather_table_rows: bad shape (B <= 256)");
    GS_REQUIRE_WS("gs_gather_table_rows", ws, ws_bytes, gs_gather_table_rows_ws_bytes(B));
    hipStream_t st = (hipStream_t)stream;
    int32_t *starts = (int32_t *)ws;
    hipLaunchKernelGGL(table_starts_k, dim3(cdiv(B + 1, 64)), dim3(64), 0, st, rows, d_n_rows, B, starts);
    GS_LAUNCH_CHECK("gs_gather_table_rows/starts");
    const int nb = max_rows > 0 ? min(cdiv(max_rows, 256), 2048) : 1;
    hipLaunchKernelGGL(gather_table_k, dim3(nb), dim3(256), 0, st, rows, d_n_rows, starts, attr, B, Nmax,
                       C, cap, out, counts);
    GS_LAUNCH_CHECK("gs_gather_table_rows");
    return GS_OK;
}

size_t gs_bucket_by_pixel_ws_bytes(int B, int H, int W, int ds) { return bucket_layout(B, H, W, ds, nullptr, nullptr); }

int gs_bucket_by_pixel(const int64_t *rows, const int32_t *d_n_rows, int64_t max_rows, int B, int H, int W, int ds,
                       const float *map_points, int Nmax, int cap, float *scan_points, int32_t *scan_orig,
                       int32_t *pix_start, int32_t *tgt_pix, void *ws, size_t ws_bytes, gs_stream_t stream) {
    GS_REQUIRE(rows && d_n_rows && map_points && scan_points && scan_orig && pix_start, "gs_bucket_by_pixel: NULL argument");
    GS_REQUIRE(B > 0 && B <= 256 && H > 0 && W > 0 && ds > 0 && Nmax > 0 && cap > 0 && max_rows >= 0, "gs_bucket_by_pixel: bad shape");
    BucketWs w;
    GS_REQUIRE_WS("gs_bucket_by_pixel", ws, ws_bytes, bucket_layout(B, H, W, ds, ws, &w));
    hipStream_t st = (hipStream_t)stream;
    const int Wd = cdiv(W, ds), npix = cdiv(H, ds) * Wd;
    int32_t *starts = w.starts;
    int *cnt = w.cnt, *fill = w.fill;
    const int64_t nbins = (int64_t)B * npix;
    hipLaunchKernelGGL(tgt_init_k, dim3(min(cdiv(nbins, 256), 1024)), dim3(256), 0, st, cnt, fill, nbins, rows, d_n_rows, B, starts);
    const int nb = max_rows > 0 ? min(cdiv(max_rows, 256), 1024) : 1;
    hipLaunchKernelGGL(pix_count_k, dim3(nb), dim3(256), 0, st, rows, d_n_rows, starts, Wd, npix, ds, cnt);
    hipLaunchKernelGGL(pix_scan_k, dim3(B), dim3(1024), 0, st, cnt, npix, pix_start);
    hipLaunchKernelGGL(pix_scatter_k, dim3(nb), dim3(256), 0, st, rows, d_n_rows, starts, Wd, npix, ds, pix_start, fill, map_points,
                       Nmax, cap, scan_points, scan_orig, tgt_pix);
    GS_LAUNCH_CHECK("gs_bucket_by_pixel");
    return GS_OK;
}

size_t gs_build_icp_target_ws_bytes(int B, int H, int W, int ds) { return gs_bucket_by_pixel_ws_bytes(B, H, W, ds); }

int gs_build_icp_target(const int64_t *rows, const int32_t *d_n_rows, int64_t max_rows, int B, int H, int W, int ds,
                        const float *map_points, const float *map_normals, int Nmax, int cap, float *tgt, float *tgt_normals,
                        int32_t *counts, float *scan_points, int32_t *scan_orig, int32_t *pix_start, int32_t *tgt_index,
                        int32_t *tgt_pix, void *ws, size_t ws_bytes, gs_stream_t stream) {
    GS_REQUIRE(rows && d_n_rows && map_points && map_normals && tgt && tgt_normals && counts && scan_points && scan_orig && pix_start,
               "gs_build_icp_target: NULL argument");
    GS_REQUIRE(B > 0 && B <= 256 && H > 0 && W > 0 && ds > 0 && Nmax > 0 && cap > 0 && max_rows >= 0, "gs_build_icp_target: bad shape");
    BucketWs w;
    GS_REQUIRE_WS("gs_build_icp_target", ws, ws_bytes, bucket_layout(B, H, W, ds, ws, &w));
    hipStream_t st = (hipStream_t)stream;
    const int Wd = cdiv(W, ds), npix = cdiv(H, ds) * Wd;
    int32_t *starts = w.starts;
    int *cnt = w.cnt, *fill = w.fill;
    const int64_t nbins = (int64_t)B * npix;
    hipLaunchKernelGGL(tgt_init_k, dim3(min(cdiv(nbins, 256), 1024)), dim3(256), 0, st, cnt, fill, nbins, rows, d_n_rows, B, starts);
    const int nb = max_rows > 0 ? min(cdiv(max_rows, 256), 1024) : 1;
    hipLaunchKernelGGL(tgt_gather_count_k, dim3(nb), dim3(256), 0, st, rows, d_n_rows, starts, map_points, map_normals, B, Nmax,
                       cap, tgt, tgt_normals, counts, Wd, npix, ds, cnt, tgt_index);
    hipLaunchKernelGGL(pix_scan_k, dim3(B), dim3(1024), 0, st, cnt, npix, pix_start);
    hipLaunchKernelGGL(pix_scatter_k, dim3(nb), dim3(256), 0, st, rows, d_n_rows, starts, Wd, npix, ds, pix_start, fill, map_points,
                       Nmax, cap, scan_points, scan_orig, tgt_pix);
    GS_LAUNCH_CHECK("gs_build_icp_target");
    return GS_OK;
}

int gs_table_ds_mask(const int64_t *rows, int64_t n_rows, int ds, uint8_t *mask, gs_stream_t stream) {
    GS_REQUIRE(rows && mask && n_rows >= 0 && ds > 0, "gs_table_ds_mask: bad arguments");
    if (n_rows == 0) return GS_OK;
    hipLaunchKernelGGL(table_ds_mask_k, dim3(min(cdiv(n_rows, 256), 2048)), dim3(256), 0, (hipStream_t)stream, rows,
                       n_rows, ds, mask);
    GS_LAUNCH_CHECK("gs_table_ds_mask");
    return GS_OK;
}

}
```

gradslam_amd/csrc/slam.hip:

```cpp
#include <algorithm>
#include <chrono>
#include <mutex>
#include <stdlib.h>
#include <vector>

#include "gs_common.hpp"
#include "gs_drivers.hpp"
#include "gs_icp.hpp"

namespace gs {

struct GraphKey {
    void *ws;
    int B, capS, capT, numiters, use_grad;
    float damp, thresh, lmax, Bp, B2, nu;
    int icp_cfg;
    int H, W, ds;
    bool operator==(const GraphKey &o) const {
        return H == o.H && W == o.W && ds == o.ds && ws == o.ws && B == o.B && capS == o.capS && capT == o.capT && numiters == o.numiters && use_grad == o.use_grad &&
               damp == o.damp && thresh == o.thresh && lmax == o.lmax && Bp == o.Bp && B2 == o.B2 && nu == o.nu &&
               icp_cfg == o.icp_cfg;
    }
};
struct GraphEntry {
    GraphKey key;
    int device;
    hipGraphExec_t exec;
    unsigned long long last_use;
};
static std::mutex g_graph_mu;
static std::vector<GraphEntry> g_graphs;
static std::vector<GraphKey> g_seen_once;
static unsigned long long g_graph_clock = 0;
static int g_graph_mode = -1;
constexpr double kSlowLaunchUs = 8.0;
static int g_auto_samples = 0;
static double g_auto_min_us = 1e30;
static int g_captures = 0, g_replays = 0;
static bool graphs_allowed() {
    static const bool env_off = getenv("GS_NO_GRAPH") != nullptr, env_on = getenv("GS_GRAPH") != nullptr;
    if (profiling_enabled()) return false;
    if (g_graph_mode >= 0) return g_graph_mode != 0;
    if (env_off) return false;
    if (env_on) return true;
    return g_auto_samples >= 4 && g_auto_min_us > kSlowLaunchUs;
}

template <class Enqueue>
static int graph_replay(const GraphKey &key, hipStream_t st, Enqueue &&enqueue, bool *launched) {
    std::lock_guard<std::mutex> lock(g_graph_mu);
    int device = 0;
    (void)hipGetDevice(&device);
    GraphEntry *hit = nullptr;
    for (auto &e : g_graphs)
        if (e.device == device && e.key == key) hit = &e;
    bool seen = false;
    if (!hit) {
        for (auto &k : g_seen_once) seen = seen || (k == key);
        if (!seen) {
            if (g_seen_once.size() >= 16) g_seen_once.erase(g_seen_once.begin());
            g_seen_once.push_back(key);
        }
    }
    if (!hit && seen) {
        hipStream_t cs = nullptr;
        hipGraph_t graph = nullptr;
        hipGraphExec_t exec = nullptr;
        bool ok = hipStreamCreateWithFlags(&cs, hipStreamNonBlocking) == hipSuccess;
        ok = ok && hipStreamBeginCapture(cs, hipStreamCaptureModeThreadLocal) == hipSuccess;
        if (ok) {
            const int r = enqueue(cs);
            const hipError_t e = hipStreamEndCapture(cs, &graph);
            ok = (r == GS_OK) && e == hipSuccess && graph != nullptr;
        }
        ok = ok && hipGraphInstantiate(&exec, graph, nullptr, nullptr, 0) == hipSuccess;
        if (graph) (void)hipGraphDestroy(graph);
        if (cs) (void)hipStreamDestroy(cs);
        if (ok) {
            if (g_graphs.size() >= 8) {
                size_t v = 0;
                for (size_t i = 1; i < g_graphs.size(); ++i)
                    if (g_graphs[i].last_use < g_graphs[v].last_use) v = i;
                (void)hipGraphExecDestroy(g_graphs[v].exec);
                g_graphs.erase(g_graphs.begin() + v);
            }
            g_graphs.push_back(GraphEntry{key, device, exec, 0});
            hit = &g_graphs.back();
            ++g_captures;
        } else {
            (void)hipGetLastError();
        }
    }
    if (hit) {
        hit->last_use = ++g_graph_clock;
        ++g_replays;
        GS_HIP(hipGraphLaunch(hit->exec, st), "gs_slam_localize/graph");
        *launched = true;
    }
    return GS_OK;
}

template <class Enqueue>
static int eager_timed(int launches, Enqueue &&enqueue) {
    const auto t0 = std::chrono::steady_clock::now();
    const int rc = enqueue();
    if (rc) return rc;
    const double us = std::chrono::duration<double, std::micro>(std::chrono::steady_clock::now() - t0).count();
    std::lock_guard<std::mutex> lock(g_graph_mu);
    if (g_auto_samples < 64) {
        ++g_auto_samples;
        g_auto_min_us = std::min(g_auto_min_us, us / launches);
    }
    return GS_OK;
}

__global__ void compose_k(const float *__restrict__ T, const float *__restrict__ P, int B, float *__restrict__ out) {
    const int b = blockIdx.x * blockDim.x + threadIdx.x;
    if (b >= B) return;
    compose44(T + 16 * b, P + 16 * b, out + 16 * b);
}

__global__ void eye4_k(float *__restrict__ T, int B) {
    const int i = blockIdx.x * blockDim.x + threadIdx.x;
    if (i < 16 * B) T[i] = ((i % 16) % 5 == 0) ? 1.0f : 0.0f;
}

struct LocWs {
    float *src;
    int32_t *src_pix;
    float *scan;
    int32_t *scan_orig;
    int32_t *pix_start;
    int32_t *ns;
    int64_t *rows;
    int32_t *nrows;
    float *tgt, *tnrm;
    int32_t *nt;
    float *T;
    float *eye;
    float *cam;
    void *sub;
    size_t sub_bytes;
};

static inline int target_cap(int Nmax) {
    int c = 1024;
    while (c < Nmax && c < (1 << 30)) c <<= 1;
    return c;
}

static size_t loc_layout(int B, int H, int W, int ds, int Nmax, void *ws, LocWs *out) {
    const int capS = cdiv(H, ds) * cdiv(W, ds), capT = target_cap(Nmax);
    Carve c{(char *)ws};
    LocWs scratch, &w = out ? *out : scratch;
    w.src = c.take<float>((size_t)B * capS * 12); w.ns = c.take<int32_t>((size_t)B * 4);
    w.src_pix = c.take<int32_t>((size_t)B * capS * 4); w.scan = c.take<float>((size_t)B * capT * 12);
    w.scan_orig = c.take<int32_t>((size_t)B * capT * 4); w.pix_start = c.take<int32_t>((size_t)B * (capS + 1) * 4);
    w.rows = c.take<int64_t>((size_t)B * capT * 32); w.nrows = c.take<int32_t>(4);
    w.tgt = c.take<float>((size_t)B * capT * 12); w.tnrm = c.take<float>((size_t)B * capT * 12); w.nt = c.take<int32_t>((size_t)B * 4);
    w.T = c.take<float>((size_t)B * 64); w.eye = c.take<float>((size_t)B * 64); w.cam = c.take<float>((size_t)B * 128);
    w.sub_bytes = std::max({gs_downsample_frame_ws_bytes(H, W, ds), gs_project_active_ws_bytes(B, Nmax), gs_gather_table_rows_ws_bytes(B),
                            gs_bucket_by_pixel_ws_bytes(B, H, W, ds), gs_icp_ws_bytes(capS, capT), project_target1_ws_bytes(H, W, ds, Nmax)});
    w.sub = c.take(w.sub_bytes);
    return c.off;
}

static int g_fused_setup = getenv("GS_FUSED_SETUP") ? atoi(getenv("GS_FUSED_SETUP")) : 1;
static inline bool fused_front(int B, int H, int W, int ds) {
    return g_fused_setup != 0 && B == 1 && (int64_t)cdiv(H, ds) * cdiv(W, ds) <= kBucketPixMax;
}

static int enqueue_front(const float *depth, const float *gvertex, const float *intrinsics, const float *prev_poses, int B, int H, int W,
                         int ds, const float *map_points, const float *map_normals, const int32_t *map_counts, int Nmax, const LocWs &w,
                         float *src, int32_t *src_pix, int32_t *ns, int32_t *nt, int32_t *tgt_index, bool compute_maps, float *vertex,
                         float *normal, float *gvertex_out, float *gnormal, float *cam_out, hipStream_t st) {
    const int capS = cdiv(H, ds) * cdiv(W, ds), capT = target_cap(Nmax);
    const DsJob frame{depth, gvertex, src, src_pix, ns};
    int rc;
    if (fused_front(B, H, W, ds))
        return project_front1(compute_maps ? depth : nullptr, map_points, map_counts, Nmax, prev_poses, intrinsics, H, W, ds, map_normals,
                              capT, vertex, normal, gvertex_out, gnormal, cam_out, (int32_t *)w.rows, w.tgt, w.tnrm, nt, tgt_index, w.scan,
                              w.scan_orig, w.pix_start, frame, w.sub, w.sub_bytes, st);
    if (compute_maps &&
        (rc = vertex_normal_maps_cam(depth, intrinsics, prev_poses, B, H, W, vertex, normal, gvertex_out, gnormal, cam_out, st))) return rc;
    if (B == 1)
        return project_target1(map_points, map_counts, Nmax, prev_poses, intrinsics, H, W, ds, map_normals, capT, w.rows, w.nrows, w.tgt,
                               w.tnrm, nt, w.scan, w.scan_orig, w.pix_start, tgt_index, nullptr, w.sub, w.sub_bytes, st, &frame);
    if ((rc = gs_downsample_frame(depth, gvertex, nullptr, nullptr, B, H, W, ds, capS, src, nullptr, nullptr, src_pix, ns, w.sub,
                                  w.sub_bytes, (gs_stream_t)st))) return rc;
    if ((rc = gs_project_active(map_points, map_counts, B, Nmax, prev_poses, intrinsics, H, W, ds, w.rows, w.nrows, w.sub, w.sub_bytes,
                                (gs_stream_t)st))) return rc;
    return gs_build_icp_target(w.rows, w.nrows, (int64_t)B * Nmax, B, H, W, ds, map_points, map_normals, Nmax, capT, w.tgt, w.tnrm, nt,
                               w.scan, w.scan_orig, w.pix_start, tgt_index, nullptr, w.sub, w.sub_bytes, (gs_stream_t)st);
}

static inline gs_icp_hints loc_hints(const LocWs &w, const int32_t *src_pix, int b, int H, int W, int ds, int capS, int capT,
                                     const float *pose, const float *intrinsics) {
    return gs_icp_hints{w.scan + (size_t)b * capT * 3, w.scan_orig + (size_t)b * capT, src_pix + (size_t)b * capS,
                        w.pix_start + (size_t)b * (capS + 1), nullptr, cdiv(W, ds), cdiv(H, ds), pose, intrinsics, ds};
}

struct FuseWs {
    float *gV, *gN, *alpha;
    void *state;
    int32_t *ctr;
    int32_t *appended;
    int *totals;
    void *sub;
    size_t sub_bytes;
};
constexpr int kCtrWords = 64;
static size_t fuse_layout(int B, int H, int W, int Nmax, void *ws, FuseWs *out) {
    const size_t npix = (size_t)B * H * W;
    Carve c{(char *)ws};
    FuseWs scratch, &w = out ? *out : scratch;
    w.gV = c.take<float>(npix * 12); w.gN = c.take<float>(npix * 12); w.alpha = c.take<float>(npix * 4);
    w.state = c.take(fusion_corr_state_bytes(B, H, W, Nmax));
    w.ctr = c.take<int32_t>((size_t)(kCtrWords + 2 * 64) * 4);
    w.appended = w.ctr + kCtrWords; w.totals = (int *)(w.ctr + kCtrWords + 64);
    w.sub_bytes = append_scratch_bytes((int64_t)H * W);
    w.sub = c.take(w.sub_bytes);
    return c.off;
}

struct FuseBwdWs {
    float *V, *N, *gV, *gN, *alpha, *g_alpha;
    void *cws;
};
static size_t fuse_bwd_layout(int B, int H, int W, void *ws, FuseBwdWs *out) {
    const size_t npix = (size_t)B * H * W;
    Carve c{(char *)ws};
    FuseBwdWs scratch, &w = out ? *out : scratch;
    w.V = c.take<float>(npix * 12); w.N = c.take<float>(npix * 12); w.gV = c.take<float>(npix * 12); w.gN = c.take<float>(npix * 12);
    w.alpha = c.take<float>(npix * 4); w.g_alpha = c.take<float>(npix * 4);
    w.cws = c.take(append_scratch_bytes((int64_t)H * W));
    c.take(256);
    return c.off;
}

struct AggWs {
    float *gV, *gN;
    int32_t *overflow, *appended;
    size_t counter_bytes;
    void *cws;
};
static size_t agg_layout(int B, int H, int W, void *ws, AggWs *out) {
    const size_t npix = (size_t)B * H * W;
    Carve c{(char *)ws};
    AggWs scratch, &w = out ? *out : scratch;
    w.gV = c.take<float>(npix * 12); w.gN = c.take<float>(npix * 12);
    const size_t counters = c.off;
    w.overflow = c.take<int32_t>(4); w.appended = c.take<int32_t>((size_t)B * 4);
    w.counter_bytes = c.off - counters;
    w.cws = c.take(append_scratch_bytes((int64_t)H * W));
    return c.off;
}

__global__ void fuse_stats_k(const int32_t *__restrict__ nrows, const int32_t *__restrict__ ucnt, const int32_t *__restrict__ overflow,
                             const float *__restrict__ max_dot, const int32_t *__restrict__ appended, int B,
                             int32_t *__restrict__ stats) {
    if (threadIdx.x == 0) {
        stats[0] = *nrows; stats[1] = *ucnt; stats[2] = *overflow; stats[3] = __float_as_int(*max_dot);
    }
    if ((int)threadIdx.x < B) stats[4 + threadIdx.x] = appended[threadIdx.x];
}

struct LocTape {
    float *src;
    int32_t *src_pix;
    int32_t *ns, *nt;
    int32_t *tgt_index;
    float *T;
    char *icp;
    size_t icp_bytes;
};
static size_t loc_tape_layout(int B, int H, int W, int ds, int Nmax, int numiters, int grad_lm, void *tape, LocTape *out) {
    const int capS = cdiv(H, ds) * cdiv(W, ds), capT = target_cap(Nmax);
    Carve c{(char *)tape};
    LocTape scratch, &t = out ? *out : scratch;
    t.src = c.take<float>((size_t)B * capS * 12); t.src_pix = c.take<int32_t>((size_t)B * capS * 4);
    t.ns = c.take<int32_t>((size_t)B * 4); t.nt = c.take<int32_t>((size_t)B * 4);
    t.tgt_index = c.take<int32_t>((size_t)B * capT * 4); t.T = c.take<float>((size_t)B * 64);
    t.icp_bytes = align_up(gs_icp_tape_bytes(capS, numiters, grad_lm), 256);
    t.icp = c.take<char>((size_t)B * t.icp_bytes);
    return c.off;
}

struct LocBwdWs {
    float *tgt, *tnrm, *g_tgt, *g_nrm;
    float *g_src;
    float *g_T, *g_init, *eye;
    void *sub;
    size_t sub_bytes;
};
static size_t loc_bwd_layout(bool det, int B, int H, int W, int ds, int Nmax, int numiters, int grad_lm, void *ws, LocBwdWs *out) {
    const int capS = cdiv(H, ds) * cdiv(W, ds), capT = target_cap(Nmax);
    Carve c{(char *)ws};
    LocBwdWs scratch, &w = out ? *out : scratch;
    w.tgt = c.take<float>((size_t)capT * 12); w.tnrm = c.take<float>((size_t)capT * 12);
    w.g_tgt = c.take<float>((size_t)capT * 12); w.g_nrm = c.take<float>((size_t)capT * 12);
    w.g_src = c.take<float>((size_t)capS * 12);
    w.g_T = c.take<float>((size_t)B * 64); w.g_init = c.take<float>((size_t)B * 64); w.eye = c.take<float>((size_t)B * 64);
    w.sub_bytes = det ? gs_icp_backward_det_ws_bytes(capS, capT, numiters, grad_lm) : gs_icp_backward_ws_bytes(capS);
    w.sub = c.take(w.sub_bytes);
    return c.off;
}

__global__ void compose_bwd_k(const float *__restrict__ T, const float *__restrict__ P, const float *__restrict__ gO, int B,
                              float *__restrict__ gT, float *__restrict__ gP) {
    const int b = blockIdx.x * blockDim.x + threadIdx.x;
    if (b >= B) return;
    const float *a = T + 16 * b, *p = P + 16 * b, *g = gO + 16 * b;
    float *ga = gT + 16 * b, *gp = gP + 16 * b;
    for (int i = 0; i < 3; ++i) {
        for (int k = 0; k < 3; ++k) ga[4 * i + k] = ((g[4 * i] * p[4 * k] + g[4 * i + 1] * p[4 * k + 1]) + g[4 * i + 2] * p[4 * k + 2]) + g[4 * i + 3] * p[4 * k + 3];
        ga[4 * i + 3] = g[4 * i + 3];
    }
    for (int k = 0; k < 3; ++k)
        for (int j = 0; j < 4; ++j) gp[4 * k + j] = (a[k] * g[j] + a[4 + k] * g[4 + j]) + a[8 + k] * g[8 + j];
    for (int j = 0; j < 4; ++j) { ga[12 + j] = 0.0f; gp[12 + j] = 0.0f; }
}

__global__ void regather_k(const int32_t *__restrict__ tgt_index, const int32_t *__restrict__ nt, int capT,
                           const float *__restrict__ map_points, const float *__restrict__ map_normals, int Nmax,
                           float *__restrict__ tgt, float *__restrict__ tnrm) {
    const int b = blockIdx.y, n = min(nt[b], capT);
    for (int k = blockIdx.x * blockDim.x + threadIdx.x; k < n; k += gridDim.x * blockDim.x) {
        const int64_t srcI = (int64_t)b * Nmax + tgt_index[(int64_t)b * capT + k], dst = (int64_t)b * capT + k;
        st3(tgt, dst, ld3(map_points, srcI));
        st3(tnrm, dst, ld3(map_normals, srcI));
    }
}

__global__ void scatter_grads_k(const float *__restrict__ g_src, const int32_t *__restrict__ src_pix, const int32_t *__restrict__ ns,
                                int capS, int Wd, int ds, int H, int W, float *__restrict__ g_gvertex ,
                                const float *__restrict__ g_tgt, const float *__restrict__ g_nrm,
                                const int32_t *__restrict__ tgt_index, const int32_t *__restrict__ nt, int capT,
                                float *__restrict__ g_map_points, float *__restrict__ g_map_normals , int accumulate) {
    const int n_s = min(*ns, capS), n_t = min(*nt, capT);
    const int stride = gridDim.x * blockDim.x;
    for (int i = blockIdx.x * blockDim.x + threadIdx.x; i < n_s; i += stride) {
        const int pix = src_pix[i];
        const int64_t at = (int64_t)(pix / Wd) * ds * W + (int64_t)(pix % Wd) * ds;
        st3(g_gvertex, at, ld3(g_src, i));
    }
    for (int k = blockIdx.x * blockDim.x + threadIdx.x; k < n_t; k += stride) {
        const int64_t at = tgt_index[k];
        f3 gp = g_map_points ? ld3(g_tgt, k) : f3{0, 0, 0}, gq = g_map_normals ? ld3(g_nrm, k) : f3{0, 0, 0};
        if (accumulate) {
            if (g_map_points) { const f3 o = ld3(g_map_points, at); gp = f3{o.x + gp.x, o.y + gp.y, o.z + gp.z}; }
            if (g_map_normals) { const f3 o = ld3(g_map_normals, at); gq = f3{o.x + gq.x, o.y + gq.y, o.z + gq.z}; }
        }
        if (g_map_points) st3(g_map_points, at, gp);
        if (g_map_normals) st3(g_map_normals, at, gq);
    }
}

}

using namespace gs;

extern "C" {

void gs_set_graph_mode(int mode) { g_graph_mode = mode; }

void gs_set_fused_setup(int on) { g_fused_setup = on; }

int gs_graph_stats(double *out4) {
    GS_REQUIRE(out4, "gs_graph_stats: NULL argument");
    std::lock_guard<std::mutex> lock(g_graph_mu);
    out4[0] = g_auto_samples; out4[1] = g_auto_min_us; out4[2] = g_captures; out4[3] = g_replays;
    return GS_OK;
}

int gs_compose_poses(const float *T, const float *P, int B, float *out, gs_stream_t stream) {
    GS_REQUIRE(T && P && out && B > 0, "gs_compose_poses: bad arguments");
    hipLaunchKernelGGL(compose_k, dim3(cdiv(B, 64)), dim3(64), 0, (hipStream_t)stream, T, P, B, out);
    GS_LAUNCH_CHECK("gs_compose_poses");
    return GS_OK;
}

size_t gs_slam_localize_ws_bytes(int B, int H, int W, int ds, int Nmax) {
    if (B <= 0 || H <= 0 || W <= 0 || ds <= 0 || Nmax <= 0) return 0;
    return loc_layout(B, H, W, ds, Nmax, nullptr, nullptr);
}

int gs_slam_localize(const float *depth, const float *intrinsics, const float *prev_poses, int B, int H, int W, int ds,
                     const float *map_points, const float *map_normals, const int32_t *map_counts, int Nmax,
                     int use_grad_lm, int numiters, float damp, float dist_thresh, float lambda_max, float Bp, float B2,
                     float nu, float *vertex, float *normal, float *gvertex, float *gnormal, float *out_poses, void *ws,
                     size_t ws_bytes, gs_stream_t stream) {
    GS_REQUIRE(depth && intrinsics && prev_poses && map_points && map_normals && map_counts && gvertex && out_poses,
               "gs_slam_localize: NULL argument (gvertex is required, the other maps are optional)");
    GS_REQUIRE(B > 0 && H >= 2 && W >= 2 && ds > 0 && Nmax > 0 && numiters >= 0, "gs_slam_localize: bad shape");
    GS_REQUIRE_WS("gs_slam_localize", ws, ws_bytes, gs_slam_localize_ws_bytes(B, H, W, ds, Nmax));
    hipStream_t st = (hipStream_t)stream;
    LocWs w;
    loc_layout(B, H, W, ds, Nmax, ws, &w);
    const int capS = cdiv(H, ds) * cdiv(W, ds), capT = target_cap(Nmax);
    int rc;
    if ((rc = enqueue_front(depth, gvertex, intrinsics, prev_poses, B, H, W, ds, map_points, map_normals, map_counts, Nmax, w, w.src,
                            w.src_pix, w.ns, w.nt, nullptr, true, vertex, normal, gvertex, gnormal, w.cam, st))) return rc;
    auto enqueue_loops = [&](hipStream_t s, bool fold_compose) -> int {
        for (int b = 0; b < B; ++b) {
            const gs_icp_hints hints = loc_hints(w, w.src_pix, b, H, W, ds, capS, capT, w.cam + 32 * b, w.cam + 32 * b + 16);
            const int r = icp_localize_run(use_grad_lm, w.src + (size_t)b * capS * 3, w.ns + b, capS, w.tgt + (size_t)b * capT * 3,
                                           w.tnrm + (size_t)b * capT * 3, w.nt + b, capT, numiters, damp, dist_thresh, lambda_max, Bp,
                                           B2, nu, &hints, w.T + 16 * b, w.sub, w.sub_bytes, s, nullptr, 0,
                                           fold_compose ? prev_poses + 16 * b : nullptr, fold_compose ? out_poses + 16 * b : nullptr);
            if (r) return r;
        }
        return GS_OK;
    };
    bool launched = false;
    if (graphs_allowed() && numiters > 0) {
        const GraphKey key{ws, B, capS, capT, numiters, use_grad_lm, damp, dist_thresh, lambda_max, Bp, B2, nu,
                           icp_config_stamp(), H, W, ds};
        if ((rc = graph_replay(key, st, [&](hipStream_t cs) { return enqueue_loops(cs, false); }, &launched))) return rc;
    }
    if (!launched) {
        if (numiters > 0)
            return eager_timed(B * ((use_grad_lm ? 2 * numiters : numiters + 1) + 2), [&] { return enqueue_loops(st, true); });
        if ((rc = enqueue_loops(st, false))) return rc;
    }
    return gs_compose_poses(w.T, prev_poses, B, out_poses, stream);
}

size_t gs_pointfusion_update_ws_bytes(int B, int H, int W, int Nmax) {
    if (B <= 0 || H <= 0 || W <= 0 || Nmax <= 0) return 0;
    return fuse_layout(B, H, W, Nmax, nullptr, nullptr);
}

static int pointfusion_update_impl(const float *depth, const float *rgb, const float *intrinsics, const float *poses, int B, int H, int W,
                                   float *map_points, float *map_normals, float *map_colors, float *map_ccounts, int32_t *map_counts,
                                   int Nmax, float dist_th, float dot_th, float sigma, int32_t *stats, void *ws, size_t ws_bytes,
                                   gs_stream_t stream, void *tape, const char *name) {
    GS_REQUIRE(depth && rgb && intrinsics && poses && map_points && map_normals && map_colors && map_ccounts && map_counts,
               "%s: NULL argument", name);
    GS_REQUIRE(B > 0 && B <= 60 && H >= 2 && W >= 2 && Nmax > 0, "%s: bad shape", name);
    GS_REQUIRE_WS(name, ws, ws_bytes, gs_pointfusion_update_ws_bytes(B, H, W, Nmax));
    hipStream_t st = (hipStream_t)stream;
    FuseWs w;
    fuse_layout(B, H, W, Nmax, ws, &w);
    int rc;
    unsigned long long *pix_key; unsigned int *pix_n;
    fusion_corr_init_ptrs(w.state, B, H, W, Nmax, &pix_key, &pix_n);
    if ((rc = vertex_normal_maps_fusion(depth, intrinsics, poses, B, H, W, w.gV, w.gN, w.alpha, sigma, 1e-7f, pix_key, pix_n, w.ctr,
                                        kCtrWords + 2 * 64, st))) return rc;
    if ((rc = fusion_correspond(w.state, map_points, map_normals, map_ccounts, map_counts, B, Nmax, poses, intrinsics, H, W, w.gV, w.gN,
                                dist_th, dot_th, w.ctr, st))) return rc;
    if (tape && (rc = fusion_tape_record(w.state, tape, B, H, W, Nmax, map_counts, map_points, map_normals, map_colors, map_ccounts, st)))
        return rc;
    if ((rc = fusion_merge_corr(w.state, w.ctr, w.gV, w.gN, rgb, w.alpha, B, H, W, Nmax, map_counts, map_points, map_normals, map_colors,
                                map_ccounts, st))) return rc;
    const int64_t HW = (int64_t)H * W;
    for (int b = 0; b < B; ++b) {
        const float *src[4] = {w.gV + b * HW * 3, w.gN + b * HW * 3, rgb + b * HW * 3, w.alpha + b * HW};
        float *dst[4] = {map_points + (size_t)b * Nmax * 3, map_normals + (size_t)b * Nmax * 3, map_colors + (size_t)b * Nmax * 3,
                         map_ccounts + (size_t)b * Nmax};
        const int widths[4] = {3, 3, 3, 1};
        if ((rc = fusion_append_corr(w.state, B, H, W, Nmax, b, depth, src, widths, dst, map_counts + b, Nmax, w.totals + b, w.sub, st)))
            return rc;
    }
    if ((rc = fusion_finish(w.state, B, H, W, Nmax, w.ctr, map_counts, w.totals, Nmax, w.appended, stats, st))) return rc;
    if (tape && (rc = fusion_tape_appended(tape, B, H, W, w.appended, st))) return rc;
    return GS_OK;
}

int gs_pointfusion_update(const float *depth, const float *rgb, const float *intrinsics, const float *poses, int B, int H, int W,
                          float *map_points, float *map_normals, float *map_colors, float *map_ccounts, int32_t *map_counts,
                          int Nmax, float dist_th, float dot_th, float sigma, int32_t *stats, void *ws, size_t ws_bytes,
                          gs_stream_t stream) {
    return pointfusion_update_impl(depth, rgb, intrinsics, poses, B, H, W, map_points, map_normals, map_colors, map_ccounts, map_counts,
                                   Nmax, dist_th, dot_th, sigma, stats, ws, ws_bytes, stream, nullptr, "gs_pointfusion_update");
}

size_t gs_pointfusion_update_tape_bytes(int B, int H, int W) {
    if (B <= 0 || H <= 0 || W <= 0) return 0;
    return fusion_tape_bytes(B, H, W);
}

int gs_pointfusion_update_taped(const float *depth, const float *rgb, const float *intrinsics, const float *poses, int B, int H, int W,
                                float *map_points, float *map_normals, float *map_colors, float *map_ccounts, int32_t *map_counts,
                                int Nmax, float dist_th, float dot_th, float sigma, int32_t *stats, void *tape, size_t tape_bytes,
                                void *ws, size_t ws_bytes, gs_stream_t stream) {
    GS_REQUIRE_TAPE("gs_pointfusion_update_taped", tape, tape_bytes, gs_pointfusion_update_tape_bytes(B, H, W), GS_ERR_INVALID_ARG);
    return pointfusion_update_impl(depth, rgb, intrinsics, poses, B, H, W, map_points, map_normals, map_colors, map_ccounts, map_counts,
                                   Nmax, dist_th, dot_th, sigma, stats, ws, ws_bytes, stream, tape, "gs_pointfusion_update_taped");
}

size_t gs_pointfusion_update_backward_ws_bytes(int B, int H, int W) {
    if (B <= 0 || H <= 0 || W <= 0) return 0;
    return fuse_bwd_layout(B, H, W, nullptr, nullptr);
}

int gs_pointfusion_update_backward(const float *depth, const float *rgb, const float *intrinsics, const float *poses, int B, int H,
                                   int W, float *map_points, float *map_normals, float *map_colors, float *map_ccounts,
                                   int32_t *map_counts, int Nmax, float sigma, const void *tape, size_t tape_bytes, float *G_points,
                                   float *G_normals, float *G_colors, float *G_ccounts, float *g_vertex, float *g_gvertex,
                                   float *g_gnormal, float *g_rgb, void *ws, size_t ws_bytes, gs_stream_t stream) {
    const char *name = "gs_pointfusion_update_backward";
    GS_REQUIRE(depth && rgb && intrinsics && poses && map_points && map_normals && map_colors && map_ccounts && map_counts && tape &&
                   G_points && G_normals && G_colors && G_ccounts && g_vertex && g_gvertex && g_gnormal && g_rgb, "%s: NULL argument", name);
    GS_REQUIRE(B > 0 && B <= 60 && H >= 2 && W >= 2 && Nmax > 0, "%s: bad shape", name);
    GS_REQUIRE_TAPE(name, tape, tape_bytes, gs_pointfusion_update_tape_bytes(B, H, W), GS_ERR_INVALID_ARG);
    GS_REQUIRE_WS(name, ws, ws_bytes, gs_pointfusion_update_backward_ws_bytes(B, H, W));
    hipStream_t st = (hipStream_t)stream;
    const size_t npix = (size_t)B * H * W;
    FuseBwdWs w;
    fuse_bwd_layout(B, H, W, ws, &w);
    int rc;
    if ((rc = gs_vertex_normal_maps(depth, intrinsics, poses, B, 1, H, W, w.V, w.N, w.gV, w.gN, stream))) return rc;
    if ((rc = gs_get_alpha(w.V, (int64_t)npix, sigma, 1e-7f, w.alpha, stream))) return rc;
    if ((rc = fusion_update_reverse(tape, B, H, W, Nmax, depth, w.gV, w.gN, rgb, w.alpha, map_points, map_normals, map_colors, map_ccounts,
                                    map_counts, G_points, G_normals, G_colors, G_ccounts, g_gvertex, g_gnormal, g_rgb, w.g_alpha, w.cws,
                                    st))) return rc;
    GS_HIP(hipMemsetAsync(g_vertex, 0, npix * 12, st), name);
    return gs_get_alpha_backward(w.V, (int64_t)npix, sigma, 1e-7f, w.g_alpha, g_vertex, stream);
}

size_t gs_aggregate_update_ws_bytes(int B, int H, int W) {
    if (B <= 0 || H <= 0 || W <= 0) return 0;
    return agg_layout(B, H, W, nullptr, nullptr);
}

int gs_aggregate_update(const float *depth, const float *rgb, const float *intrinsics, const float *poses, int B, int H, int W,
                        float *map_points, float *map_normals, float *map_colors, int32_t *map_counts, int Nmax, int32_t *stats,
                        void *ws, size_t ws_bytes, gs_stream_t stream) {
    const char *name = "gs_aggregate_update";
    GS_REQUIRE(depth && rgb && intrinsics && poses && map_points && map_normals && map_colors && map_counts, "%s: NULL argument", name);
    GS_REQUIRE(B > 0 && B <= 60 && H >= 2 && W >= 2 && Nmax > 0, "%s: bad shape", name);
    GS_REQUIRE_WS(name, ws, ws_bytes, gs_aggregate_update_ws_bytes(B, H, W));
    hipStream_t st = (hipStream_t)stream;
    AggWs w;
    agg_layout(B, H, W, ws, &w);
    GS_HIP(hipMemsetAsync(w.overflow, 0, w.counter_bytes, st), name);
    int rc;
    if ((rc = gs_vertex_normal_maps(depth, intrinsics, poses, B, 1, H, W, nullptr, nullptr, w.gV, w.gN, stream))) return rc;
    const int64_t HW = (int64_t)H * W;
    for (int b = 0; b < B; ++b) {
        const float *src[3] = {w.gV + b * HW * 3, w.gN + b * HW * 3, rgb + b * HW * 3};
        float *dst[3] = {map_points + (size_t)b * Nmax * 3, map_normals + (size_t)b * Nmax * 3, map_colors + (size_t)b * Nmax * 3};
        const int widths[3] = {3, 3, 3};
        if ((rc = append_valid_pixels(3, depth + b * HW, HW, src, widths, dst, map_counts + b, Nmax, w.appended + b, w.overflow, w.cws,
                                      st))) return rc;
    }
    if (stats) {
        hipLaunchKernelGGL(fuse_stats_k, dim3(1), dim3(64), 0, st, w.overflow, w.overflow, w.overflow, (const float *)w.overflow, w.appended, B,
                           stats);
        GS_LAUNCH_CHECK(name);
    }
    return GS_OK;
}

// ... 114 lines not shown
```

gradslam_amd/ops.py:

```python
import math
from typing import Optional, Tuple

import torch

from . import _native as nv
from ._native import call, ptr, require_hip, stream, workspace, ws_bytes


def _f32c(t: Optional[torch.Tensor]) -> Optional[torch.Tensor]:
    if t is None:
        return None
    if t.dtype != torch.float32:
        t = t.float()
    return t.contiguous()


def deterministic() -> bool:
    return torch.are_deterministic_algorithms_enabled()


def dev_int(value: int, device) -> torch.Tensor:
    return torch.full((1,), int(value), dtype=torch.int32, device=device)


# ... 311 lines not shown
        dev = src.device
        z = lambda t, n: torch.zeros(n, dtype=torch.float32, device=dev) if t is None else _f32c(t).reshape(-1)
        gout = torch.cat([z(gH, 36), z(gg, 6), z(ge, 1)])
        g_src = torch.zeros_like(src_c)
        g_tgt = torch.zeros_like(tgt_c)
        g_nrm = torch.zeros_like(nrm_c)
        ns, nt = src_c.shape[0], tgt_c.shape[0]
        if deterministic():
            ws = workspace(ws_bytes("gs_icp_linearize_backward_det_ws_bytes", ns, nt), dev, "linearize_bwd_det")
            d_ns, d_nt = dev_int(ns, dev), dev_int(nt, dev)
            call("gs_icp_linearize_backward_det", ptr(src_c), ptr(d_ns), ns, ptr(tgt_c), ptr(nrm_c), ptr(d_nt), nt, ptr(best), _thresh(ctx.dist_thresh), ptr(gout), ptr(g_src), ptr(g_tgt), ptr(g_nrm), ptr(ws), ws.numel(), stream())
        else:
            call("gs_icp_linearize_backward", ptr(src_c), ptr(dev_int(ns, dev)), ns, ptr(tgt_c), ptr(nrm_c), ptr(best),
                 _thresh(ctx.dist_thresh), ptr(gout), ptr(g_src), ptr(g_tgt), ptr(g_nrm), stream())
        return g_src, g_tgt, g_nrm, None, None


def icp_linearize(src, tgt, nrm, best, dist_thresh):
    return _LinearizeFn.apply(src, tgt, nrm, best, dist_thresh)


def icp_rows_raw(src, tgt, nrm, best, dist_thresh):
    src, tgt, nrm = _f32c(src), _f32c(tgt), _f32c(nrm)
    dev = src.device
    n = src.shape[0]
    A = torch.empty((n, 6), dtype=torch.float32, device=dev)
    b = torch.empty(n, dtype=torch.float32, device=dev)
    keep = torch.empty(n, dtype=torch.uint8, device=dev)
    call("gs_icp_rows", ptr(src), ptr(dev_int(n, dev)), n, ptr(tgt), ptr(nrm), ptr(best), _thresh(dist_thresh), ptr(A),
         ptr(b), ptr(keep), stream())
    return A, b, keep


class _TransformFn(torch.autograd.Function):

    @staticmethod
    def forward(ctx, pts, T):
        p, Tc = _f32c(pts), _f32c(T)
        out = torch.empty_like(p)
        call("gs_transform_points", ptr(p), ptr(dev_int(p.shape[0], p.device)), p.shape[0], ptr(Tc), ptr(out), stream())
        ctx.save_for_backward(p, Tc)
        return out

    @staticmethod
    def backward(ctx, g):
        p, T = ctx.saved_tensors
        g = _f32c(g)
        Tt = torch.zeros_like(T)
        Tt[:3, :3] = T[:3, :3].t()
        Tt[3, 3] = 1.0
        gp = torch.empty_like(p)
        call("gs_transform_points", ptr(g), ptr(dev_int(p.shape[0], p.device)), p.shape[0], ptr(Tt.contiguous()), ptr(gp), stream())
        gT = torch.zeros_like(T)
        gT[:3, :3] = g.t() @ p
        gT[:3, 3] = g.sum(0)
        return gp, gT


def transform_points(pts: torch.Tensor, T: torch.Tensor) -> torch.Tensor:
    require_hip(pts, T, op="transform_points")
    return _TransformFn.apply(pts, T)


def icp_device_loop(src, tgt, nrm, init_T, numiters, damp, dist_thresh, grad_params=None, want_trace=False,
                    want_best=False):
    require_hip(src, tgt, nrm, init_T, op="icp")
    src, tgt, nrm, init_T = _f32c(src.detach()), _f32c(tgt.detach()), _f32c(nrm.detach()), _f32c(init_T.detach())
    dev = src.device
    ns, nt = src.shape[0], tgt.shape[0]
    if ns == 0 or nt == 0:
        raise ValueError("ICP needs non-empty source and target clouds (got {} and {} points)".format(ns, nt))
    T = torch.empty((4, 4), dtype=torch.float32, device=dev)
    best = torch.empty(ns, dtype=torch.int64, device=dev) if want_best else None
    trace = torch.zeros((max(numiters, 1), 48), dtype=torch.float32, device=dev) if want_trace else None
    ws = workspace(ws_bytes("gs_icp_ws_bytes", ns, nt), dev, "icp")
    d_ns, d_nt = dev_int(ns, dev), dev_int(nt, dev)
    if grad_params is None:
        call("gs_icp_point_to_plane", ptr(src), ptr(d_ns), ns, ptr(tgt), ptr(nrm), ptr(d_nt), nt, ptr(init_T),
             int(numiters), float(damp), _thresh(dist_thresh), None, ptr(T), ptr(best), ptr(trace), ptr(ws), ws.numel(), stream())
    else:
        lmax, Bp, B2, nu = grad_params
        call("gs_icp_point_to_plane_grad", ptr(src), ptr(d_ns), ns, ptr(tgt), ptr(nrm), ptr(d_nt), nt, ptr(init_T),
             int(numiters), float(damp), _thresh(dist_thresh), float(lmax), float(Bp), float(B2), float(nu), None, ptr(T),
             ptr(best), ptr(trace), ptr(ws), ws.numel(), stream())
    return T, best, trace


def _grad_lm(grad_params):
    lmax, Bp, B2, nu = grad_params if grad_params is not None else (2.0, 1.0, 1.0, 200.0)
    return (1 if grad_params is not None else 0), float(lmax), float(Bp), float(B2), float(nu)


class _IcpLoopFn(torch.autograd.Function):

    @staticmethod
    def forward(ctx, src, tgt, nrm, init_T, numiters, damp, dist_thresh, grad_params):
        src, tgt, nrm, init_T = _f32c(src.detach()), _f32c(tgt.detach()), _f32c(nrm.detach()), _f32c(init_T.detach())
        dev = src.device
        ns, nt = src.shape[0], tgt.shape[0]
        if ns == 0 or nt == 0:
            raise ValueError("ICP needs non-empty source and target clouds (got {} and {} points)".format(ns, nt))
        grad_lm, lmax, Bp, B2, nu = _grad_lm(grad_params)
        T = torch.empty((4, 4), dtype=torch.float32, device=dev)
        best = torch.empty(ns, dtype=torch.int64, device=dev)
        tape = torch.empty(ws_bytes("gs_icp_tape_bytes", ns, int(numiters), grad_lm), dtype=torch.uint8, device=dev)
        ws = workspace(ws_bytes("gs_icp_ws_bytes", ns, nt), dev, "icp")
        d_ns, d_nt = dev_int(ns, dev), dev_int(nt, dev)
        call("gs_icp_point_to_plane_taped", ptr(src), ptr(d_ns), ns, ptr(tgt), ptr(nrm), ptr(d_nt), nt, ptr(init_T),
             int(numiters), float(damp), _thresh(dist_thresh), grad_lm, lmax, Bp, B2, nu, None,
             ptr(T), ptr(best), ptr(tape), tape.numel(), ptr(ws), ws.numel(), stream())
        ctx.save_for_backward(src, tgt, nrm, init_T, tape, d_ns, d_nt)
        ctx.cfg = (int(numiters), _thresh(dist_thresh), grad_lm, lmax, Bp, B2, nu)
        ctx.mark_non_differentiable(best)
        return T, best

    @staticmethod
    def backward(ctx, gT, _gbest):
        src, tgt, nrm, init_T, tape, d_ns, d_nt = ctx.saved_tensors
        numiters, thresh, grad_lm, lmax, Bp, B2, nu = ctx.cfg
        dev = src.device
        ns, nt = src.shape[0], tgt.shape[0]
        gT = _f32c(gT)
        need_tgt, need_nrm = ctx.needs_input_grad[1], ctx.needs_input_grad[2]
        g_src = torch.empty_like(src)
        g_tgt = torch.empty_like(tgt) if need_tgt else None
        g_nrm = torch.empty_like(nrm) if need_nrm else None
        g_init = torch.empty((4, 4), dtype=torch.float32, device=dev)
        if deterministic():
            entry = "gs_icp_point_to_plane_backward_det"
            ws = workspace(ws_bytes("gs_icp_backward_det_ws_bytes", ns, nt, numiters, grad_lm), dev, "icp_bwd_det")
        else:
            entry = "gs_icp_point_to_plane_backward"
            ws = workspace(ws_bytes("gs_icp_backward_ws_bytes", ns), dev, "icp_bwd")
        call(entry, ptr(src), ptr(d_ns), ns, ptr(tgt), ptr(nrm), ptr(d_nt), nt, ptr(init_T), numiters, thresh,
             grad_lm, lmax, Bp, B2, nu, ptr(tape), tape.numel(), ptr(gT), ptr(g_src), ptr(g_tgt), ptr(g_nrm), ptr(g_init),
             ptr(ws), ws.numel(), stream())
        return g_src, g_tgt, g_nrm, g_init, None, None, None, None


def icp_loop_autograd(src, tgt, nrm, init_T, numiters, damp, dist_thresh, grad_params=None):
    require_hip(src, tgt, nrm, init_T, op="icp")
    return _IcpLoopFn.apply(src, tgt, nrm, init_T, numiters, damp, dist_thresh, grad_params)


def slam_localize_raw(depth, K, prev_poses, map_points, map_normals, map_counts_i32, ds, numiters, damp, dist_thresh,
                      grad_params=None, out=None, want_maps=True):
    require_hip(depth, K, prev_poses, map_points, map_normals, map_counts_i32, op="slam_localize")
    depth, K, prev = _f32c(depth.detach()), _f32c(K.detach()), _f32c(prev_poses.detach())
    mp, mn = _f32c(map_points.detach()), _f32c(map_normals.detach())
    B, _, H, W = depth.shape[:4]
    Nmax = mp.shape[1]
    dev = depth.device
    mk = lambda: torch.empty((B, 1, H, W, 3), dtype=torch.float32, device=dev)
    V, N, gV = (mk() if want_maps else None), (mk() if want_maps else None), mk()
    if out is None:
        out = torch.empty((B, 1, 4, 4), dtype=torch.float32, device=dev)
    elif not (out.is_contiguous() and out.dtype == torch.float32 and out.numel() == 16 * B and out.device == dev):
        raise ValueError("slam_localize: `out` must be a contiguous float32 (B,1,4,4) tensor on the inputs' device")
    ws = workspace(ws_bytes("gs_slam_localize_ws_bytes", B, H, W, int(ds), Nmax), dev, "localize")
    grad_lm, lmax, Bp, B2, nu = _grad_lm(grad_params)
    call("gs_slam_localize", ptr(depth), ptr(K), ptr(prev), B, H, W, int(ds), ptr(mp), ptr(mn), ptr(map_counts_i32), Nmax,
         grad_lm, int(numiters), float(damp), _thresh(dist_thresh), lmax, Bp, B2, nu, ptr(V), ptr(N), ptr(gV), None, ptr(out),
         ptr(ws), ws.numel(), stream())
    return out, V, N


def slam_localize_taped_raw(gV, depth, K, prev_poses, map_points, map_normals, map_counts_i32, ds, numiters, damp, dist_thresh,
                            grad_params=None):
    require_hip(gV, depth, K, prev_poses, map_points, map_normals, map_counts_i32, op="slam_localize")
    gV, depth, K, prev = _f32c(gV.detach()), _f32c(depth.detach()), _f32c(K.detach()), _f32c(prev_poses.detach())
    mp, mn = _f32c(map_points.detach()), _f32c(map_normals.detach())
    B, _, H, W = depth.shape[:4]
    Nmax = mp.shape[1]
    dev = depth.device
    grad_lm, lmax, Bp, B2, nu = _grad_lm(grad_params)
    out = torch.empty((B, 1, 4, 4), dtype=torch.float32, device=dev)
    tape = torch.empty(ws_bytes("gs_slam_localize_tape_bytes", B, H, W, int(ds), Nmax, int(numiters), grad_lm),
                       dtype=torch.uint8, device=dev)
    ws = workspace(ws_bytes("gs_slam_localize_ws_bytes", B, H, W, int(ds), Nmax), dev, "localize")
    call("gs_slam_localize_taped", ptr(depth), ptr(gV), ptr(K), ptr(prev), B, H, W, int(ds), ptr(mp), ptr(mn),
         ptr(map_counts_i32), Nmax, grad_lm, int(numiters), float(damp), _thresh(dist_thresh), lmax, Bp, B2, nu, ptr(out),
         ptr(tape), tape.numel(), ptr(ws), ws.numel(), stream())
    return out, tape


def slam_localize_backward_raw(prev_poses, map_points, map_normals, nmax, H, W, ds, numiters, dist_thresh, grad_params, tape,
                               g_poses, g_gV, g_map_points, g_map_normals, g_prev, accumulate):
    B, dev = prev_poses.shape[0], prev_poses.device
    ds, numiters = int(ds), int(numiters)
    grad_lm, lmax, Bp, B2, nu = _grad_lm(grad_params)
    g_poses = _f32c(g_poses)
    if deterministic():
        det, size = "_det", ws_bytes("gs_slam_localize_backward_det_ws_bytes", B, H, W, ds, nmax, numiters, grad_lm)
    else:
        det, size = "", ws_bytes("gs_slam_localize_backward_ws_bytes", B, H, W, ds, nmax)
    ws = workspace(size, dev, "localize_bwd" + det)
    call("gs_slam_localize_backward" + det, ptr(prev_poses), B, H, W, ds, ptr(map_points), ptr(map_normals), nmax, grad_lm,
         numiters, _thresh(dist_thresh), lmax, Bp, B2, nu, ptr(tape), tape.numel(), ptr(g_poses), ptr(g_gV), ptr(g_map_points),
         ptr(g_map_normals), ptr(g_prev), int(accumulate), ptr(ws), ws.numel(), stream())


class _LocalizeFn(torch.autograd.Function):

    @staticmethod
    def forward(ctx, gV, depth, K, prev_poses, mp, mn, counts_i32, ds, numiters, damp, dist_thresh, grad_params):
        prev, mp, mn = _f32c(prev_poses.detach()), _f32c(mp.detach()), _f32c(mn.detach())
        out, tape = slam_localize_taped_raw(gV, depth, K, prev, mp, mn, counts_i32, ds, numiters, damp, dist_thresh, grad_params)
        ctx.save_for_backward(prev, mp, mn, tape)
        ctx.cfg = (depth.shape[2], depth.shape[3], ds, numiters, dist_thresh, grad_params)
        return out

    @staticmethod
    def backward(ctx, g_out):
        prev, mp, mn, tape = ctx.saved_tensors
        H, W = ctx.cfg[:2]
        B, dev = prev.shape[0], prev.device
        g_gV = torch.empty((B, 1, H, W, 3), dtype=torch.float32, device=dev)
        g_mp = torch.empty_like(mp) if ctx.needs_input_grad[4] else None
        g_mn = torch.empty_like(mn) if ctx.needs_input_grad[5] else None
        g_prev = torch.empty((B, 1, 4, 4), dtype=torch.float32, device=dev)
        slam_localize_backward_raw(prev, mp, mn, mp.shape[1], *ctx.cfg, tape, g_out, g_gV, g_mp, g_mn, g_prev, 0)
        return g_gV, None, None, g_prev, g_mp, g_mn, None, None, None, None, None, None


def slam_localize_autograd(gV, depth, K, prev_poses, map_points, map_normals, map_counts_i32, ds, numiters, damp, dist_thresh,
                           grad_params=None):
    return _LocalizeFn.apply(gV, depth, K, prev_poses, map_points, map_normals, map_counts_i32, ds, numiters, damp, dist_thresh,
                             grad_params)


def _pointfusion_update_args(depth, rgb, K, poses, map_points, map_normals, map_colors, map_ccounts, map_counts_i32, nmax=None):
    require_hip(depth, rgb, K, poses, map_points, map_normals, map_colors, map_ccounts, map_counts_i32, op="pointfusion_update")
    for name, x in (("map_points", map_points), ("map_normals", map_normals), ("map_colors", map_colors),
                    ("map_ccounts", map_ccounts), ("depth", depth), ("rgb", rgb)):
        if not (x.is_contiguous() and x.dtype == torch.float32):
            raise ValueError("pointfusion_update: {} must be contiguous float32 (it is updated / read in place)".format(name))
    B, H, W = depth.shape[:3]
    nmax = map_points.shape[1] if nmax is None else int(nmax)
    held = K, poses = _f32c(K), _f32c(poses)
    return B, H, W, nmax, held, (ptr(depth), ptr(rgb), ptr(K), ptr(poses), B, H, W, ptr(map_points), ptr(map_normals),
                                 ptr(map_colors), ptr(map_ccounts), ptr(map_counts_i32), nmax)


def pointfusion_update_raw(depth, rgb, K, poses, map_points, map_normals, map_colors, map_ccounts, map_counts_i32, dist_th,
                           dot_th, sigma, stats=None):
    B, H, W, Nmax, held, prefix = _pointfusion_update_args(depth, rgb, K, poses, map_points, map_normals, map_colors, map_ccounts,
                                                           map_counts_i32)
    ws = workspace(ws_bytes("gs_pointfusion_update_ws_bytes", B, H, W, Nmax), depth.device, "fusion_step")
    call("gs_pointfusion_update", *prefix, float(dist_th), float(dot_th), float(sigma), ptr(stats), ptr(ws), ws.numel(), stream())


def pointfusion_update_taped_raw(depth, rgb, K, poses, map_points, map_normals, map_colors, map_ccounts, map_counts_i32, dist_th,
                                 dot_th, sigma, stats=None):
    B, H, W, Nmax, held, prefix = _pointfusion_update_args(depth, rgb, K, poses, map_points, map_normals, map_colors, map_ccounts,
                                                           map_counts_i32)
    tape = torch.empty(ws_bytes("gs_pointfusion_update_tape_bytes", B, H, W), dtype=torch.uint8, device=depth.device)
    ws = workspace(ws_bytes("gs_pointfusion_update_ws_bytes", B, H, W, Nmax), depth.device, "fusion_step")
    call("gs_pointfusion_update_taped", *prefix, float(dist_th), float(dot_th), float(sigma), ptr(stats), ptr(tape), tape.numel(),
         ptr(ws), ws.numel(), stream())
    return tape


def pointfusion_update_backward_raw(depth, rgb, K, poses, map_points, map_normals, map_colors, map_ccounts, map_counts_i32, nmax,
                                    sigma, tape, G_points, G_normals, G_colors, G_ccounts, g_V, g_gV, g_gN, g_rgb):
    B, H, W, nmax, held, prefix = _pointfusion_update_args(depth, rgb, K, poses, map_points, map_normals, map_colors, map_ccounts,
                                                           map_counts_i32, nmax)
    ws = workspace(ws_bytes("gs_pointfusion_update_backward_ws_bytes", B, H, W), depth.device, "fusion_bwd")
    call("gs_pointfusion_update_backward", *prefix, float(sigma), ptr(tape), tape.numel(), ptr(G_points), ptr(G_normals),
         ptr(G_colors), ptr(G_ccounts), ptr(g_V), ptr(g_gV), ptr(g_gN), ptr(g_rgb), ptr(ws), ws.numel(), stream())


def aggregate_update_raw(depth, rgb, K, poses, map_points, map_normals, map_colors, map_counts_i32, stats=None):
    require_hip(depth, rgb, K, poses, map_points, map_normals, map_colors, map_counts_i32, op="aggregate_update")
    for name, x in (("map_points", map_points), ("map_normals", map_normals), ("map_colors", map_colors), ("depth", depth), ("rgb", rgb)):
        if not (x.is_contiguous() and x.dtype == torch.float32):
            raise ValueError("aggregate_update: {} must be contiguous float32 (it is updated / read in place)".format(name))
    B, H, W = depth.shape[:3]
    K, poses = _f32c(K), _f32c(poses)
    ws = workspace(ws_bytes("gs_aggregate_update_ws_bytes", B, H, W), depth.device, "aggregate_step")
    call("gs_aggregate_update", ptr(depth), ptr(rgb), ptr(K), ptr(poses), B, H, W, ptr(map_points), ptr(map_normals),
         ptr(map_colors), ptr(map_counts_i32), map_points.shape[1], ptr(stats), ptr(ws), ws.numel(), stream())


def fusion_similar_raw(rows, n_rows_dev, max_rows, gV, gN, map_points, map_normals, dist_th, dot_th):
    gV, gN, mp, mn = _f32c(gV), _f32c(gN), _f32c(map_points), _f32c(map_normals)
    H, W = gV.shape[2:4]
    dev = gV.device
    keep = torch.zeros(max(max_rows, 1), dtype=torch.uint8, device=dev)
    max_dot = torch.zeros(1, dtype=torch.float32, device=dev)
    call("gs_fusion_similar", ptr(rows), ptr(n_rows_dev), max_rows, ptr(gV), ptr(gN), H, W, ptr(mp), ptr(mn),
         mp.shape[1], float(dist_th), float(dot_th), ptr(keep), ptr(max_dot), stream())
    return keep, max_dot


def fusion_unique_raw(rows, keep, n_rows_dev, max_rows, gV, map_points, map_ccounts):
    gV, mp, cc = _f32c(gV), _f32c(map_points), _f32c(map_ccounts)
    B, _, H, W = gV.shape[:4]
    dev = gV.device
    out = torch.empty((B * H * W, 4), dtype=torch.int64, device=dev)
    cnt = torch.zeros(1, dtype=torch.int32, device=dev)
    ws = workspace(ws_bytes("gs_fusion_unique_ws_bytes", B, H, W), dev, "unique")
    call("gs_fusion_unique", ptr(rows), ptr(keep), ptr(n_rows_dev), max_rows, ptr(gV), B, H, W, ptr(mp), ptr(cc),
         mp.shape[1], ptr(out), ptr(cnt), ptr(ws), ws.numel(), stream())
    return out, cnt


def fusion_merge_raw(rows, n_rows_dev, max_rows, gV, gN, rgb, alpha, counts_dev, mp, mn, mc, cc):
    B, _, H, W = gV.shape[:4]
    Nmax = mp.shape[1]
    dev = gV.device
    op, on, oc, occ = (torch.empty_like(x) for x in (mp, mn, mc, cc))
    ws = workspace(ws_bytes("gs_fusion_merge_ws_bytes", B, Nmax), dev, "merge")
    call("gs_fusion_merge", ptr(rows), ptr(n_rows_dev), max_rows, ptr(gV), ptr(gN), ptr(rgb), ptr(alpha), B, H, W, Nmax,
         ptr(counts_dev), ptr(mp), ptr(mn), ptr(mc), ptr(cc), ptr(op), ptr(on), ptr(oc), ptr(occ), ptr(ws), ws.numel(),
         stream())
# ... 976 lines not shown
```

Before: 6303 frames/s.

## Compute source points from depth, precompute bucket ranks, and hoist loads in ICP kernels

After: 6323 frames/s, median of 6. About the same (+0.3%).

```diff
diff --git a/gradslam_amd/csrc/gs_drivers.hpp b/gradslam_amd/csrc/gs_drivers.hpp
--- a/gradslam_amd/csrc/gs_drivers.hpp
+++ b/gradslam_amd/csrc/gs_drivers.hpp
@@ -10,6 +10,8 @@
 int vertex_normal_maps_fusion(const float *depth, const float *intrinsics, const float *poses, int B, int H, int W, float *gvertex,
                               float *gnormal, float *alpha, float sigma, float eps, unsigned long long *pix_key, unsigned int *pix_n,
                               int32_t *zero, int n_zero, hipStream_t st);
+int downsample_frame_from_depth(const float *depth, const float *intrinsics, const float *poses, int B, int H, int W, int ds, int cap,
+                                float *out_points, int32_t *out_pix, int32_t *counts, void *ws, size_t ws_bytes, hipStream_t st);
 
 constexpr int kBucketPixMax = 24 * 1024;
 size_t project_target1_ws_bytes(int H, int W, int ds, int Nmax);
diff --git a/gradslam_amd/csrc/gs_icp_loop.hpp b/gradslam_amd/csrc/gs_icp_loop.hpp
--- a/gradslam_amd/csrc/gs_icp_loop.hpp
+++ b/gradslam_amd/csrc/gs_icp_loop.hpp
@@ -641,19 +641,35 @@
 }
 
 __global__ __launch_bounds__(SUPER * CHUNK) void icp_prepare_k(IcpState *S, const float *__restrict__ init_T, float damp,
-                                                              const float *__restrict__ tgt, const int32_t *__restrict__ d_nt,
+                                                              const float *__restrict__ tgt, const int32_t *__restrict__ d_nt, int max_nt,
                                                               float *__restrict__ boxes, float *__restrict__ sboxes,
                                                               LoopConst lc, LoopConst *__restrict__ lc_out, float *__restrict__ part0,
                                                               float *__restrict__ part1, int rows_written, int rows_read) {
     static_assert(SUPER * CHUNK == 1024, "one block per super-box");
+    __shared__ float wb[16][6];
+    __shared__ float raw[48];
+    const int ns = *lc.d_ns, nt = *d_nt;
+    const int j = blockIdx.x * (SUPER * CHUNK) + threadIdx.x;
+    const bool have_cam = lc.hints.cam_pose && lc.hints.cam_K && lc.hints.ds > 0;
+    int pix0 = 0;
+    if (lc.cells && lc.hints.src_pix) pix0 = lc.hints.src_pix[min(j, lc.cells_stride - 1)];
+    const f3 p = ld3(tgt, min(j, max_nt - 1));
+    float w0 = 0.0f;
+    {
+        const int t = threadIdx.x & 15;
+        const float *from = threadIdx.x < 16 ? lc.hints.cam_pose : threadIdx.x < 32 ? lc.hints.cam_K : init_T;
+        const bool want = blockIdx.x == 0 && threadIdx.x < 48 && from && (threadIdx.x >= 32 || have_cam);
+        if (want) w0 = from[t];
+    }
+    asm volatile("" ::"v"(pix0), "v"(p.x), "v"(p.y), "v"(p.z), "v"(w0));
+    if (blockIdx.x == 0 && threadIdx.x < 48) raw[threadIdx.x] = w0;
     for (int q = rows_written * NACC + blockIdx.x * blockDim.x + threadIdx.x; q < rows_read * NACC; q += gridDim.x * blockDim.x) {
         part0[q] = 0.0f; part1[q] = 0.0f;
     }
-    __shared__ float wb[16][6];
     if (blockIdx.x == 0 && threadIdx.x < sizeof(LoopConst) / 4) {
         int v = reinterpret_cast<const int *>(&lc)[threadIdx.x];
-        if (threadIdx.x == offsetof(LoopConst, ns) / 4) v = *lc.d_ns;
-        if (threadIdx.x == offsetof(LoopConst, nt) / 4) v = *lc.d_nt;
+        if (threadIdx.x == offsetof(LoopConst, ns) / 4) v = ns;
+        if (threadIdx.x == offsetof(LoopConst, nt) / 4) v = nt;
         if (threadIdx.x == offsetof(LoopConst, tile_points) / 4) {
             atomicAdd(&g_loop_counts[0], 1u);
             if (lc.grid_variant) atomicAdd(&g_loop_counts[1], 1u);
@@ -662,15 +678,15 @@
         reinterpret_cast<int *>(lc_out)[threadIdx.x] = v;
     }
     if (lc.cells) {
-        const int n = *lc.d_ns;
         int32_t *pix = lc.cells + 2 * (size_t)lc.cells_stride;
-        for (int i = blockIdx.x * blockDim.x + threadIdx.x; i < lc.cells_stride; i += gridDim.x * blockDim.x)
-            pix[i] = (i < n && lc.hints.src_pix) ? lc.hints.src_pix[i] : 0;
+        if (j < lc.cells_stride) pix[j] = (j < ns && lc.hints.src_pix) ? pix0 : 0;
+        for (int i = j + gridDim.x * blockDim.x; i < lc.cells_stride; i += gridDim.x * blockDim.x)
+            pix[i] = (i < ns && lc.hints.src_pix) ? lc.hints.src_pix[i] : 0;
     }
     if (blockIdx.x == 0) {
         __syncthreads();
-        if (threadIdx.x == 0 && lc.hints.cam_pose && lc.hints.cam_K && lc.hints.ds > 0) {
-            const float *T = lc.hints.cam_pose, *K = lc.hints.cam_K;
+        if (threadIdx.x == 0 && have_cam) {
+            const float *T = raw, *K = raw + 16;
             const Cam c = make_cam(T, K);
             for (int q = 0; q < 9; ++q) lc_out->cam.R[q] = c.R[q];
             for (int q = 0; q < 3; ++q) lc_out->cam.T[q] = c.tinv[q];
@@ -683,7 +699,7 @@
     }
     if (threadIdx.x == 0 && blockIdx.x == 0) {
         for (int i = 0; i < 16; ++i) {
-            const float v = init_T ? init_T[i] : ((i % 5 == 0) ? 1.0f : 0.0f);
+            const float v = init_T ? raw[32 + i] : ((i % 5 == 0) ? 1.0f : 0.0f);
             S->T[i] = v; S->dT[i] = v;
         }
         for (int i = 0; i < 44; ++i) S->cur[i] = 0.0f;
@@ -693,14 +709,9 @@
         S->b_cur = 1; S->b_first = 0;
         S->it = 0;
     }
-    const int nt = *d_nt;
-    const int j = blockIdx.x * (SUPER * CHUNK) + threadIdx.x;
     if (blockIdx.x * (SUPER * CHUNK) >= nt) return;
     float lo[3] = {INFINITY, INFINITY, INFINITY}, hi[3] = {-INFINITY, -INFINITY, -INFINITY};
-    if (j < nt) {
-        const f3 p = ld3(tgt, j);
-        lo[0] = hi[0] = p.x; lo[1] = hi[1] = p.y; lo[2] = hi[2] = p.z;
-    }
+    if (j < nt) { lo[0] = hi[0] = p.x; lo[1] = hi[1] = p.y; lo[2] = hi[2] = p.z; }
 #pragma unroll
     for (int a = 0; a < 3; ++a) {
 #pragma unroll
diff --git a/gradslam_amd/csrc/gs_maps.hpp b/gradslam_amd/csrc/gs_maps.hpp
--- a/gradslam_amd/csrc/gs_maps.hpp
+++ b/gradslam_amd/csrc/gs_maps.hpp
@@ -21,6 +21,15 @@
     const float x = k.a * (float)w + k.c;
     const float y = k.e * (float)h + k.f;
     return f3{(x * d) * m, (y * d) * m, (1.0f * d) * m};
+}
+
+__device__ __forceinline__ f3 global_vertex_of(const float *__restrict__ T, f3 v, float d) {
+    const float m = d > 0.0f ? 1.0f : 0.0f;
+    const f3 g = xform(T, v);
+    return f3{g.x * m, g.y * m, g.z * m};
+}
+__device__ __forceinline__ f3 global_vertex_from_depth(const float *__restrict__ K, const float *__restrict__ T, int h, int w, float d) {
+    return global_vertex_of(T, vertex_of(load_kinv(K), h, w, d), d);
 }
 
 struct VnExtra {
@@ -102,10 +111,7 @@
     if (gvertex || gnormal) {
         if (poses) {
             const float *T = poses + 16 * (int64_t)bl;
-            if (gvertex) {
-                f3 g = xform(T, v);
-                st3(gvertex, pix, f3{g.x * m, g.y * m, g.z * m});
-            }
+            if (gvertex) st3(gvertex, pix, global_vertex_of(T, v, d));
             if (gnormal) {
                 st3(gnormal, pix,
                     f3{dot3_fma(T[0], T[1], T[2], n.x, n.y, n.z), dot3_fma(T[4], T[5], T[6], n.x, n.y, n.z),
diff --git a/gradslam_amd/csrc/gs_project.hpp b/gradslam_amd/csrc/gs_project.hpp
--- a/gradslam_amd/csrc/gs_project.hpp
+++ b/gradslam_amd/csrc/gs_project.hpp
@@ -1,6 +1,7 @@
 #pragma once
 
 #include "gs_common.hpp"
+#include "gs_maps.hpp"
 
 namespace gs {
 
@@ -68,11 +69,12 @@
     float *op, *on, *oc;
     int32_t *opix;
     int W, Wd, ds;
+    const float *depth = nullptr, *K = nullptr, *T = nullptr;
     __device__ void operator()(int64_t i, int64_t pos) const {
         const int r = (int)(i / Wd), c = (int)(i - (int64_t)r * Wd);
         const int64_t pix = (int64_t)(r * ds) * W + c * ds;
         if (opix) opix[pos] = (int32_t)i;
-        if (op) st3(op, pos, ld3(gv, pix));
+        if (op) st3(op, pos, depth ? global_vertex_from_depth(K, T, r * ds, c * ds, depth[pix]) : ld3(gv, pix));
         if (on) st3(on, pos, ld3(gn, pix));
         if (oc) st3(oc, pos, ld3(rgb, pix));
     }
diff --git a/gradslam_amd/csrc/icp.hip b/gradslam_amd/csrc/icp.hip
--- a/gradslam_amd/csrc/icp.hip
+++ b/gradslam_amd/csrc/icp.hip
@@ -312,8 +312,24 @@
 #ifdef GS_DIAG_STAMPS
     if (g_diag && threadIdx.x == 0) g_diag[0] = wall_clock64();
 #endif
-    if (threadIdx.x < kWords) reinterpret_cast<int *>(&st)[threadIdx.x] = reinterpret_cast<const int *>(Sg)[threadIdx.x];
-    reduce_partials(partials, nblocks, acc);
+    __shared__ float right[16];
+    static_assert(kWords <= 1024 - 16, "the last sixteen lanes carry the pose");
+    constexpr int kRight0 = 1024 - 16;
+    const int g = threadIdx.x >> 5;
+    float a[RP_LOADS];
+    rp_issue(partials, nblocks, g, a);
+    int st_w = 0;
+    float right_w = 0.0f;
+    if (threadIdx.x < kWords) st_w = reinterpret_cast<const int *>(Sg)[threadIdx.x];
+    if (compose_out && threadIdx.x >= kRight0) right_w = compose_right[threadIdx.x - kRight0];
+    float v = rp_sum(a, nblocks, g, 0.0f);
+    for (int b0 = g + 32 * RP_LOADS; b0 < nblocks; b0 += 32 * RP_LOADS) {
+        rp_issue(partials, nblocks, b0, a);
+        v = rp_sum(a, nblocks, b0, v);
+    }
+    if (threadIdx.x < kWords) reinterpret_cast<int *>(&st)[threadIdx.x] = st_w;
+    if (threadIdx.x >= kRight0) right[threadIdx.x - kRight0] = right_w;
+    rp_finish(v, acc);
     if (rec && threadIdx.x < kWords) reinterpret_cast<int *>(rec)[REC_STATE + threadIdx.x] = reinterpret_cast<const int *>(Sg)[threadIdx.x];
 #ifdef GS_DIAG_STAMPS
     if (g_diag && threadIdx.x == 0) g_diag[1] = wall_clock64();
@@ -328,7 +344,7 @@
         reinterpret_cast<int *>(Sg)[threadIdx.x] = v;
         if (rec) reinterpret_cast<int *>(rec)[REC_WORDS + REC_STATE + threadIdx.x] = v;
     }
-    if (compose_out && threadIdx.x == 0) compose44(st.T, compose_right, compose_out);
+    if (compose_out && threadIdx.x == 0) compose44(st.T, right, compose_out);
 }
 
 static int icp_run(bool grad, const float *src, const int32_t *d_ns, int max_ns, const float *tgt, const float *nrm,
@@ -370,7 +386,7 @@
     LoopConst lc{src, tgt, nrm, w.boxes, w.sboxes, d_ns, d_nt, trace, out_T, hints, gp, thresh, 0, 0, cert_off, tile_points,
                  grid_search ? 1 : 0, CamK{}, 0, w.cells, max_ns};
     hipLaunchKernelGGL(icp_prepare_k, dim3(cdiv(max_nt, SUPER * CHUNK)), dim3(SUPER * CHUNK), 0, st, w.S[0], init_T, damp,
-                       hints.scan_points ? hints.scan_points : tgt, d_nt, w.boxes, w.sboxes, lc, w.lc, w.partials[0], w.partials[1], lb,
+                       hints.scan_points ? hints.scan_points : tgt, d_nt, max_nt, w.boxes, w.sboxes, lc, w.lc, w.partials[0], w.partials[1], lb,
                        std::max(lb, 32 * RP_LOADS));
     GS_LAUNCH_CHECK(name);
     int cur = 0;
diff --git a/gradslam_amd/csrc/maps.hip b/gradslam_amd/csrc/maps.hip
--- a/gradslam_amd/csrc/maps.hip
+++ b/gradslam_amd/csrc/maps.hip
@@ -547,3 +547,23 @@
 }
 
 }
+
+namespace gs {
+int downsample_frame_from_depth(const float *depth, const float *intrinsics, const float *poses, int B, int H, int W, int ds, int cap,
+                                float *out_points, int32_t *out_pix, int32_t *counts, void *ws, size_t ws_bytes, hipStream_t st) {
+    const char *name = "gs_slam_localize/source";
+    GS_REQUIRE(depth && intrinsics && poses && out_points && counts && B > 0 && H > 0 && W > 0 && ds > 0, "%s: bad arguments", name);
+    const int Hd = cdiv(H, ds), Wd = cdiv(W, ds);
+    GS_REQUIRE(cap >= Hd * Wd, "%s: cap (%d) < ceil(H/ds)*ceil(W/ds) (%d)", name, cap, Hd * Wd);
+    GS_REQUIRE_WS(name, ws, ws_bytes, gs_downsample_frame_ws_bytes(H, W, ds));
+    const int64_t HW = (int64_t)H * W;
+    for (int b = 0; b < B; ++b) {
+        DsPred pred{depth + b * HW, W, Wd, ds};
+        DsWriter wr{nullptr, nullptr, nullptr, out_points + 3 * (int64_t)b * cap, nullptr, nullptr,
+                    out_pix ? out_pix + (int64_t)b * cap : nullptr, W, Wd, ds, depth + b * HW, intrinsics + 16 * b, poses + 16 * b};
+        int rc = compact_launch((int64_t)Hd * Wd, pred, wr, counts + b, ws, st, name);
+        if (rc != GS_OK) return rc;
+    }
+    return GS_OK;
+}
+}
diff --git a/gradslam_amd/csrc/project.hip b/gradslam_amd/csrc/project.hip
--- a/gradslam_amd/csrc/project.hip
+++ b/gradslam_amd/csrc/project.hip
@@ -106,7 +106,10 @@
     __device__ void block_init(int pass, int bid, int nb) const {
         if (threadIdx.x == 0) cam_cache()[0] = make_cam(poses, Ks);
         if (pass == 0)
-            for (int i = bid * blockDim.x + threadIdx.x; i < npix; i += nb * blockDim.x) { cnt[i] = 0; fill[i] = 0; }
+            for (int i = bid * blockDim.x + threadIdx.x; i < npix; i += nb * blockDim.x) {
+                cnt[i] = 0;
+                if (fill) fill[i] = 0;
+            }
     }
     struct Item { f3 p; };
     __device__ Item fetch(int64_t i) const { return Item{ld3(points, i)}; }
@@ -141,18 +144,19 @@
     int cap;
     float *tgt, *tnrm;
     int32_t *tgt_index;
-    int32_t *row_pix;
+    int32_t *row_pix, *row_rank;
     __device__ void put(const ActivePredH::Item &it, int64_t i, int64_t pos) const {
         int h, w;
         project_point(cam_cache()[0], it.p, H, W, umax, vmax, h, w);
         const int pix = (h / ds) * Wd + (w / ds);
-        atomicAdd(cnt + pix, 1);
+        const int rank = atomicAdd(cnt + pix, 1);
         row_pix[pos] = pix;
         if (pos < cap) {
             st3(tgt, pos, it.p);
             st3(tnrm, pos, ld3(normals, i));
             if (tgt_index) tgt_index[pos] = (int32_t)i;
         }
+        row_rank[pos] = rank;
     }
     __device__ void operator()(int64_t i, int64_t pos) const { put(ActivePredH::Item{ld3(points, i)}, i, pos); }
 };
@@ -380,6 +384,11 @@
 }
 
 namespace gs {
+static inline DsWriter ds_job_writer(const DsJob &f, const float *intrinsics, const float *poses, int W, int Wd, int ds) {
+    DsWriter w{f.gvertex, nullptr, nullptr, f.out_points, nullptr, nullptr, f.out_pix, W, Wd, ds};
+    if (!f.gvertex) { w.depth = f.depth; w.K = intrinsics; w.T = poses; }
+    return w;
+}
 size_t project_target1_ws_bytes(int H, int W, int ds, int Nmax) { return front_layout(H, W, ds, Nmax, nullptr, nullptr); }
 int project_target1(const float *points, const int32_t *counts, int Nmax, const float *poses, const float *intrinsics, int H,
                     int W, int ds, const float *map_normals, int cap, int64_t *rows, int32_t *nrows, float *tgt, float *tnrm,
@@ -399,7 +408,7 @@
     if (frame) {
         const int Hd = cdiv(H, ds);
         DsPred dp{frame->depth, W, Wd, ds};
-        DsWriter dw{frame->gvertex, nullptr, nullptr, frame->out_points, nullptr, nullptr, frame->out_pix, W, Wd, ds};
+        const DsWriter dw = ds_job_writer(*frame, intrinsics, poses, W, Wd, ds);
         if (compact_blocks((int64_t)Hd * Wd) <= kSelfScanBlocks) {
             rc = compact_launch2((int64_t)Nmax, pred, wr, nrows, cws, flags, (int64_t)Hd * Wd, dp, dw, frame->count, dws, st, name);
         } else {
@@ -437,17 +446,30 @@
 
 constexpr int kBucketBlocks = 128;
 __global__ __launch_bounds__(1024) void bucket_scatter_k(const float *__restrict__ tgt, const int32_t *__restrict__ d_nt, int cap,
-                                                         const int32_t *__restrict__ row_pix, const int *__restrict__ cnt,
-                                                         int *__restrict__ fill, int npix, int32_t *__restrict__ pix_start,
+                                                         const int32_t *__restrict__ row_pix, const int32_t *__restrict__ row_rank,
+                                                         const int *__restrict__ cnt, int npix, int32_t *__restrict__ pix_start,
                                                          float *__restrict__ scan_pts, int32_t *__restrict__ scan_orig) {
+    constexpr int kPer = kBucketPixMax / 1024;
+    static_assert(kPer * 1024 == kBucketPixMax, "a whole number of counts per thread");
     __shared__ int starts[kBucketPixMax];
     __shared__ int sm[1024 / 64 + 1];
     const int nt = *d_nt;
-    for (int i = threadIdx.x; i < npix; i += 1024) starts[i] = cnt[i];
+    int c[kPer];
+#pragma unroll
+    for (int k = 0; k < kPer; ++k) c[k] = cnt[min((int)threadIdx.x + 1024 * k, npix - 1)];
     const int stride = gridDim.x * 1024;
-    int r = blockIdx.x * 1024 + threadIdx.x, pix = 0;
-    f3 p{0.0f, 0.0f, 0.0f};
-    if (r < nt) { pix = row_pix[r]; p = ld3(tgt, r); }
+    int r = blockIdx.x * 1024 + threadIdx.x;
+    const int r0 = min(r, cap - 1);
+    int pix = row_pix[r0], rank = row_rank[r0];
+    f3 p = ld3(tgt, r0);
+    asm volatile("" ::"v"(c[0]), "v"(c[1]), "v"(c[2]), "v"(c[3]), "v"(c[4]), "v"(c[5]), "v"(c[6]), "v"(c[7]), "v"(c[8]), "v"(c[9]), "v"(c[10]),
+                 "v"(c[11]), "v"(c[12]), "v"(c[13]), "v"(c[14]), "v"(c[15]), "v"(c[16]), "v"(c[17]), "v"(c[18]), "v"(c[19]), "v"(c[20]),
+                 "v"(c[21]), "v"(c[22]), "v"(c[23]), "v"(pix), "v"(rank), "v"(p.x), "v"(p.y), "v"(p.z));
+    static_assert(kPer == 24, "the asm above names every count");
+#pragma unroll
+    for (int k = 0; k < kPer; ++k)
+        if ((int)threadIdx.x + 1024 * k < npix) starts[threadIdx.x + 1024 * k] = c[k];
+    if (r >= nt) pix = 0;
     __syncthreads();
     const int per = (npix + 1023) / 1024;
     const int i0 = min(npix, (int)threadIdx.x * per), i1 = min(npix, i0 + per);
@@ -462,16 +484,16 @@
         if (threadIdx.x == 0) pix_start[npix] = total;
     }
     for (; r < nt; r += stride) {
-        const int slot = starts[pix] + atomicAdd(fill + pix, 1);
+        const int slot = starts[pix] + rank;
         const int rn = r + stride;
-        int pn = 0;
+        int pn = 0, kn = 0;
         f3 pp{0.0f, 0.0f, 0.0f};
-        if (rn < nt) { pn = row_pix[rn]; pp = ld3(tgt, rn); }
+        if (rn < nt) { pn = row_pix[rn]; kn = row_rank[rn]; pp = ld3(tgt, rn); }
         if (slot < cap) {
             st3(scan_pts, slot, p);
             scan_orig[slot] = r;
         }
-        pix = pn; p = pp;
+        pix = pn; rank = kn; p = pp;
     }
 }
 
@@ -487,13 +509,14 @@
         set_error("%s: ds-grid too large for the fused form", name);
         return GS_ERR_INVALID_ARG;
     }
-    int *cnt = w.cnt, *fill = w.fill;
+    int *cnt = w.cnt;
     unsigned char *flags = w.flags;
+    int32_t *row_rank = row_pix + cap;
     const float umax = (float)((double)W - 0.999), vmax = (float)((double)H - 0.999);
-    ActivePredH pa{points, counts, poses, intrinsics, Nmax, H, W, ds, umax, vmax, cnt, fill, npix};
-    ActiveWriterT wa{points, map_normals, H, W, ds, Wd, umax, vmax, cnt, cap, tgt, tnrm, tgt_index, row_pix};
+    ActivePredH pa{points, counts, poses, intrinsics, Nmax, H, W, ds, umax, vmax, cnt, nullptr, npix};
+    ActiveWriterT wa{points, map_normals, H, W, ds, Wd, umax, vmax, cnt, cap, tgt, tnrm, tgt_index, row_pix, row_rank};
     DsPred pb{frame.depth, W, Wd, ds};
-    DsWriter wb{frame.gvertex, nullptr, nullptr, frame.out_points, nullptr, nullptr, frame.out_pix, W, Wd, ds};
+    const DsWriter wb = ds_job_writer(frame, intrinsics, poses, W, Wd, ds);
     const int64_t nA = Nmax, nB = (int64_t)npix;
     const CompactWs cA = compact_ws(nA, false, w.map_cws);
     int *countsA = cA.counts, *countsB = compact_ws(nB, false, w.frame_cws).counts;
@@ -519,7 +542,8 @@
     }
     GS_LAUNCH_CHECK(name);
     hipLaunchKernelGGL(bucket_scatter_k, dim3(std::min(cdiv(cap, 1024), kBucketBlocks)), dim3(1024), 0, st, (const float *)tgt,
-                       (const int32_t *)nt, cap, (const int32_t *)row_pix, (const int *)cnt, fill, npix, pix_start, scan_points, scan_orig);
+                       (const int32_t *)nt, cap, (const int32_t *)row_pix, (const int32_t *)row_rank, (const int *)cnt, npix, pix_start, scan_points,
+                       scan_orig);
     GS_LAUNCH_CHECK(name);
     return GS_OK;
 }
diff --git a/gradslam_amd/csrc/slam.hip b/gradslam_amd/csrc/slam.hip
--- a/gradslam_amd/csrc/slam.hip
+++ b/gradslam_amd/csrc/slam.hip
@@ -175,7 +175,7 @@
                          float *src, int32_t *src_pix, int32_t *ns, int32_t *nt, int32_t *tgt_index, bool compute_maps, float *vertex,
                          float *normal, float *gvertex_out, float *gnormal, float *cam_out, hipStream_t st) {
     const int capS = cdiv(H, ds) * cdiv(W, ds), capT = target_cap(Nmax);
-    const DsJob frame{depth, gvertex, src, src_pix, ns};
+    const DsJob frame{depth, compute_maps ? nullptr : gvertex, src, src_pix, ns};
     int rc;
     if (fused_front(B, H, W, ds))
         return project_front1(compute_maps ? depth : nullptr, map_points, map_counts, Nmax, prev_poses, intrinsics, H, W, ds, map_normals,
@@ -186,8 +186,10 @@
     if (B == 1)
         return project_target1(map_points, map_counts, Nmax, prev_poses, intrinsics, H, W, ds, map_normals, capT, w.rows, w.nrows, w.tgt,
                                w.tnrm, nt, w.scan, w.scan_orig, w.pix_start, tgt_index, nullptr, w.sub, w.sub_bytes, st, &frame);
-    if ((rc = gs_downsample_frame(depth, gvertex, nullptr, nullptr, B, H, W, ds, capS, src, nullptr, nullptr, src_pix, ns, w.sub,
-                                  w.sub_bytes, (gs_stream_t)st))) return rc;
+    if ((rc = compute_maps ? downsample_frame_from_depth(depth, intrinsics, prev_poses, B, H, W, ds, capS, src, src_pix, ns, w.sub,
+                                                         w.sub_bytes, st)
+                           : gs_downsample_frame(depth, gvertex, nullptr, nullptr, B, H, W, ds, capS, src, nullptr, nullptr, src_pix, ns,
+                                                 w.sub, w.sub_bytes, (gs_stream_t)st))) return rc;
     if ((rc = gs_project_active(map_points, map_counts, B, Nmax, prev_poses, intrinsics, H, W, ds, w.rows, w.nrows, w.sub, w.sub_bytes,
                                 (gs_stream_t)st))) return rc;
     return gs_build_icp_target(w.rows, w.nrows, (int64_t)B * Nmax, B, H, W, ds, map_points, map_normals, Nmax, capT, w.tgt, w.tnrm, nt,
@@ -390,8 +392,8 @@
                      int use_grad_lm, int numiters, float damp, float dist_thresh, float lambda_max, float Bp, float B2,
                      float nu, float *vertex, float *normal, float *gvertex, float *gnormal, float *out_poses, void *ws,
                      size_t ws_bytes, gs_stream_t stream) {
-    GS_REQUIRE(depth && intrinsics && prev_poses && map_points && map_normals && map_counts && gvertex && out_poses,
-               "gs_slam_localize: NULL argument (gvertex is required, the other maps are optional)");
+    GS_REQUIRE(depth && intrinsics && prev_poses && map_points && map_normals && map_counts && out_poses,
+               "gs_slam_localize: NULL argument (the four maps are optional)");
     GS_REQUIRE(B > 0 && H >= 2 && W >= 2 && ds > 0 && Nmax > 0 && numiters >= 0, "gs_slam_localize: bad shape");
     GS_REQUIRE_WS("gs_slam_localize", ws, ws_bytes, gs_slam_localize_ws_bytes(B, H, W, ds, Nmax));
     hipStream_t st = (hipStream_t)stream;
@@ -399,7 +401,7 @@
     loc_layout(B, H, W, ds, Nmax, ws, &w);
     const int capS = cdiv(H, ds) * cdiv(W, ds), capT = target_cap(Nmax);
     int rc;
-    if ((rc = enqueue_front(depth, gvertex, intrinsics, prev_poses, B, H, W, ds, map_points, map_normals, map_counts, Nmax, w, w.src,
+    if ((rc = enqueue_front(depth, nullptr, intrinsics, prev_poses, B, H, W, ds, map_points, map_normals, map_counts, Nmax, w, w.src,
                             w.src_pix, w.ns, w.nt, nullptr, true, vertex, normal, gvertex, gnormal, w.cam, st))) return rc;
     auto enqueue_loops = [&](hipStream_t s, bool fold_compose) -> int {
         for (int b = 0; b < B; ++b) {
diff --git a/gradslam_amd/ops.py b/gradslam_amd/ops.py
--- a/gradslam_amd/ops.py
+++ b/gradslam_amd/ops.py
@@ -487,7 +487,7 @@
     Nmax = mp.shape[1]
     dev = depth.device
     mk = lambda: torch.empty((B, 1, H, W, 3), dtype=torch.float32, device=dev)
-    V, N, gV = (mk() if want_maps else None), (mk() if want_maps else None), mk()
+    V, N = (mk() if want_maps else None), (mk() if want_maps else None)
     if out is None:
         out = torch.empty((B, 1, 4, 4), dtype=torch.float32, device=dev)
     elif not (out.is_contiguous() and out.dtype == torch.float32 and out.numel() == 16 * B and out.device == dev):
@@ -495,7 +495,7 @@
     ws = workspace(ws_bytes("gs_slam_localize_ws_bytes", B, H, W, int(ds), Nmax), dev, "localize")
     grad_lm, lmax, Bp, B2, nu = _grad_lm(grad_params)
     call("gs_slam_localize", ptr(depth), ptr(K), ptr(prev), B, H, W, int(ds), ptr(mp), ptr(mn), ptr(map_counts_i32), Nmax,
-         grad_lm, int(numiters), float(damp), _thresh(dist_thresh), lmax, Bp, B2, nu, ptr(V), ptr(N), ptr(gV), None, ptr(out),
+         grad_lm, int(numiters), float(damp), _thresh(dist_thresh), lmax, Bp, B2, nu, ptr(V), ptr(N), None, None, ptr(out),
          ptr(ws), ws.numel(), stream())
     return out, V, N
 
```
